# rtqichen/torchdiffeq

Measured on NVIDIA B200. Metric: trajectories/sec (dopri5, batch=65536 dim=128), higher is better.
Workload: dtype f32

## Files before the change

### include/tdq.h

```cpp
#ifndef TDQ_H_
#define TDQ_H_

#include <stddef.h>
#include <stdint.h>

#ifdef __cplusplus
extern "C" {
#endif

#define TDQ_ABI_VERSION 2

#define TDQ_MAX_STAGES 16
#define TDQ_MAX_K      (TDQ_MAX_STAGES + 1)
#define TDQ_MAX_SEGS   64
#define TDQ_MAX_RANKS  16

typedef enum {
    TDQ_OK = 0,
    TDQ_ERR_INVALID = 1,
    TDQ_ERR_CUDA = 2,
    TDQ_ERR_UNSUPPORTED = 3
} tdq_status;

typedef enum { TDQ_F32 = 0, TDQ_F64 = 1 } tdq_dtype;

typedef enum {
    TDQ_RUN_OK = 0,
    TDQ_RUN_DT_UNDERFLOW = 1,
    TDQ_RUN_NONFINITE = 2,
    TDQ_RUN_MAX_STEPS = 3,
    TDQ_RUN_EXCHANGE_TIMEOUT = 4
} tdq_run_status;

typedef struct {
    int32_t n_stages;
    int32_t order;
    int32_t fsal;
    int32_t reserved;
    double alpha[TDQ_MAX_STAGES];
    double beta[TDQ_MAX_STAGES][TDQ_MAX_K];
    double c_sol[TDQ_MAX_K];
    double c_err[TDQ_MAX_K];
    double c_mid[TDQ_MAX_K];
} tdq_tableau;

typedef struct {
    int32_t dtype;
    int32_t ratio_f64;
    double rtol, atol;
    double min_step, max_step;
    double safety, ifactor, dfactor;
    double t_sign;
    int64_t max_num_steps;
    int64_t n_global;
    void *ybuf[2];
    void *kbuf[2];
    int32_t always_fit;
    int32_t reserved;
    uint64_t loop_handle;
} tdq_options;

typedef struct {
    volatile uint64_t seq;
    volatile int32_t status;
    volatile int32_t accept;
    volatile int32_t done;
    volatile int32_t out_cursor;
    volatile int64_t n_accept, n_reject;
    volatile double t0, t1, dt;
    volatile double ratio;
    volatile double att_t0, att_dt;
    volatile double next_t0, next_dt;
    volatile int32_t on_jump_t;
    volatile int32_t par;
} tdq_mailbox;

int tdq_abi_version(void);
size_t tdq_sizeof(int32_t which);
const char *tdq_last_error(void);
int tdq_device_sm_count(int *out);

int tdq_tableau_get(const char *name, tdq_tableau *out);

int tdq_mailbox_create(tdq_mailbox **host_ptr, void **dev_ptr);
int tdq_mailbox_destroy(tdq_mailbox *host_ptr);

size_t tdq_ctrl_size(void);
size_t tdq_ctrl_tstage_offset(void);
size_t tdq_ctrl_taux_offset(void);

int tdq_ctrl_init(void *ctrl_dev, const tdq_tableau *tab, const tdq_options *opt, const double *t_out_dev,
                  double t_start, int32_t n_out, void *mailbox_dev, void *stream);

int tdq_ctrl_set_step_t(void *ctrl_dev, const double *step_t_dev, int32_t n, void *stream);
int tdq_ctrl_set_jump_t(void *ctrl_dev, const double *jump_t_dev, int32_t n, void *stream);

int64_t tdq_norm_table_fill(const int64_t *seg_offsets, const int64_t *seg_lens, int32_t n_seg, int64_t n,
                            int32_t dtype, int64_t *table_host, int64_t capacity_words);
size_t tdq_norm_partials_len(size_t n, int64_t n_chunks);

int tdq_scaled_sumsq(void *ctrl_dev, int32_t dtype, const void *x, const void *x2, const void *y0,
                     const double *rtol_vec, const double *atol_vec, const int64_t *table_dev, int64_t n_chunks,
                     int32_t table_aligned, int32_t n_seg, size_t n, double *partials, double *out, void *stream);
int tdq_initial_step_h0(void *ctrl_dev, int32_t dtype, const double *d0_sumsq, const double *d1_sumsq,
                        const int64_t *seg_counts_dev, int32_t n_seg, void *stream);
int tdq_initial_step_probe(void *ctrl_dev, int32_t dtype, void *y_probe, const void *y0, const void *f0,
                           size_t n, void *stream);
int tdq_initial_step_finish(void *ctrl_dev, int32_t dtype, const double *d2_sumsq,
                            const int64_t *seg_counts_dev, int32_t n_seg, void *stream);
int tdq_set_first_step(void *ctrl_dev, double first_step, void *stream);

int tdq_prepare_attempt(void *ctrl_dev, int32_t dtype, const double *y0_nonfinite_count_dev, void *stream);

int tdq_stage_combine(void *ctrl_dev, const tdq_tableau *tab, int32_t dtype, int32_t row, void *y_out,
                      const void *y0, const void *const *k, size_t n, void *stream);

int tdq_stage_combine_final(void *ctrl_dev, const tdq_tableau *tab, int32_t dtype, void *y1_out, void *err_out,
                            const void *y0, const void *const *k, size_t n, void *stream);

int tdq_error_norm_commit(void *ctrl_dev, int32_t dtype, const void *err_pre, const void *k_last, const void *y0,
                          const void *y1, const double *rtol_vec, const double *atol_vec, const int64_t *table_dev,
                          int64_t n_chunks, int32_t table_aligned, int32_t n_seg, size_t n, double *partials,
                          double *out, void *err_over_tol_out, void *stream);
int tdq_commit_candidates(void *ctrl_dev, int32_t dtype, const void *y1, const void *k_last, size_t n, void *stream);

int tdq_controller(void *ctrl_dev, int32_t dtype, const double *norm_in, const int64_t *seg_counts_dev,
                   int32_t n_seg, const void *ratio_dev, void *stream);

int tdq_interp_fit_eval(void *ctrl_dev, const tdq_tableau *tab, int32_t dtype, const void *y1, const void *const *k,
                        void *const *coeff, void *solution, size_t n, void *stream);
int tdq_interp_eval_at(void *ctrl_dev, int32_t dtype, const void *const *coeff, const double *t_dev, void *out,
                       size_t n, void *stream);
int tdq_poly_eval(int32_t dtype, const void *const *coeff, double x, void *out, size_t n, void *stream);
int tdq_ctrl_reset_interval(void *ctrl_dev, void *stream);

int tdq_loop_create(void *body_graph, void **loop_out, uint64_t *handle_out);
int tdq_loop_launch(void *loop, void *stream);
int tdq_loop_destroy(void *loop);
int tdq_ctrl_set_loop(void *ctrl_dev, uint64_t loop_handle, void *stream);

int tdq_rk4_stage(int32_t dtype, int32_t which, void *y_out, const void *y0, const void *k1,
                  const void *k2, const void *k3, const void *k4, const void *dt_dev,
                  const int64_t *step_dev, size_t n, void *stream);
int tdq_fixed_emit(int32_t dtype, void *y0, const void *y1, void *solution,
                   const int32_t *rec_begin_dev, const int32_t *out_idx_dev, const int32_t *mode_dev,
                   const void *slope_dev, int64_t *step_dev, const void *tstage_all_dev,
                   void *tstage_cur_dev, int64_t n_steps, size_t n, void *stream);

int tdq_fixed_final_emit(int32_t dtype, int32_t which, void *y0, const void *k1, const void *k2, const void *k3,
                         const void *k4, const void *dt_dev, void *solution, const int32_t *rec_begin_dev,
                         const int32_t *out_idx_dev, const int32_t *mode_dev, const void *slope_dev, int64_t *step_dev,
                         const void *tstage_all_dev, void *tstage_cur_dev, int64_t n_steps, size_t n, void *stream);

int tdq_lincomb(int32_t dtype, void *out, const void *base, const void *const *x, const double *coefs, int32_t n_terms,
                size_t n, void *stream);

int tdq_linear_supported(int32_t dtype, int32_t width);
size_t tdq_linear_weights_bytes(int32_t width);
int tdq_linear_prepare(int32_t dtype, const void *weight, int32_t width, void *planes, void *stream);
int tdq_linear_apply(int32_t dtype, const void *y, const void *planes, int32_t width, size_t n_rows, void *k_out,
                     void *stream);
int tdq_linear_stage(void *ctrl_dev, const tdq_tableau *tab, int32_t dtype, int32_t row, void *k_out, void *y1_out,
                     void *err_out, const void *y0, const void *const *k, const void *planes, int32_t width, size_t n,
                     void *stream);

int tdq_linear_attempt_supported(const tdq_tableau *tab, int32_t dtype, int32_t width);
int tdq_linear_attempt(void *ctrl_dev, const tdq_tableau *tab, int32_t dtype, void *const *k_out, void *y1_out, void *err_out,
                       const void *y0, const void *k0, const void *planes, int32_t width, size_t n, double *partials,
                       double *norm_out, const int64_t *seg_counts_dev, int32_t store_always, void *stream);

int tdq_fixed_emit_cubic(int32_t dtype, const void *y0, const void *y1, const void *f0, const void *f1, void *solution,
                         const int32_t *out_idx_dev, const void *coef_dev, int32_t rec_lo, int32_t rec_hi, size_t n,
                         void *stream);

typedef struct { unsigned char bytes[64]; } tdq_ipc_handle;
int tdq_xchg_create(void **dev_ptr, tdq_ipc_handle *handle_out);
int tdq_xchg_open(const tdq_ipc_handle *handle, void **peer_ptr);
int tdq_xchg_close(void *peer_ptr);
int tdq_xchg_destroy(void *dev_ptr);
int tdq_ctrl_set_exchange(void *ctrl_dev, const void *const *peer_ptrs, int32_t rank, int32_t world,
                          uint64_t epoch, void *stream);

int tdq_pack_segments(int32_t dtype, void *dst, const void *const *src, const int64_t *offsets,
                      const int64_t *lens, const double *scales, int32_t n_src, void *stream);

#ifdef __cplusplus
}
#endif
#endif
```

### torchdiffeq_b200/_engine.py

```python
import ctypes as C
import time

import torch

from . import _lib

_DTYPES = {torch.float32: _lib.TDQ_F32, torch.float64: _lib.TDQ_F64}


def _stream():
    return torch.cuda.current_stream().cuda_stream


_SOLVER_STREAMS = {}


def solver_stream(device):
    idx = device.index if device.index is not None else torch.cuda.current_device()
    st = _SOLVER_STREAMS.get(idx)
    if st is None:
        st = _SOLVER_STREAMS[idx] = torch.cuda.Stream(device=idx)
    return st


class on_solver_stream:

    def __init__(self, device):
        self.device = device

    def __enter__(self):
        self.cur = torch.cuda.current_stream(self.device)
        self.s = solver_stream(self.device)
        if self.cur == self.s:
            self.ctx = None
            return self
        self.s.wait_stream(self.cur)
        self.ctx = torch.cuda.stream(self.s)
        self.ctx.__enter__()
        return self

    def __exit__(self, *exc):
        if self.ctx is not None:
            self.ctx.__exit__(*exc)
            self.cur.wait_stream(self.s)
        return False

    def publish(self, *tensors):
        if self.ctx is not None:
            for t in tensors:
                if isinstance(t, torch.Tensor) and t.is_cuda:
                    t.record_stream(self.cur)


class _RetryWithCopies(Exception):
    """func handed back a buffer it had already returned for an earlier stage of the same attempt."""


class SolverFailure(AssertionError):
    """Raised for the reference's in-loop assertions (rk_common.py:247, :286, :287)."""


class Layout:

    def __init__(self, shapes, dtype):
        self.shapes = [torch.Size(s) for s in shapes]
        self.dtype = dtype
        vec = 16 // torch.empty((), dtype=dtype).element_size()
        self.offsets, self.lens = [], []
        off = 0
        for s in self.shapes:
            n = s.numel()
            self.offsets.append(off)
            self.lens.append(n)
            off += (n + vec - 1) // vec * vec
        self.n = off
        self.n_real = sum(self.lens)

    def flatten(self, tensors, out=None):
        flat = out if out is not None else torch.zeros(self.n, dtype=self.dtype, device=tensors[0].device)
        for t, o, l in zip(tensors, self.offsets, self.lens):
            flat[o:o + l].copy_(t.reshape(-1))
        return flat

    def views(self, flat, lead=()):
        return tuple(flat[..., o:o + l].view((*lead, *s)) for o, l, s in zip(self.offsets, self.lens, self.shapes))


def pack_pieces(lib, dt_code, dtype, buf, f, pieces):
    offs, lens, scales = pieces
    srcs, keep = [], []
    for p_, l in zip(f, lens):
        if p_ is None:
            srcs.append(None)
            continue
        if p_.dtype != dtype:
            p_ = p_.to(dtype)
        p_ = p_.reshape(-1)
        if not p_.is_contiguous():
            p_ = p_.contiguous()
        if p_.numel() != l:
            raise ValueError("func returned a piece of %d elements, expected %d" % (p_.numel(), l))
        keep.append(p_)
        srcs.append(p_.data_ptr())
    n_launch = 0
    for lo in range(0, len(srcs), _lib.TDQ_MAX_SEGS):
        hi = min(lo + _lib.TDQ_MAX_SEGS, len(srcs))
        _lib.check(lib.tdq_pack_segments(
            dt_code, buf.data_ptr(), _lib.ptr_array(srcs[lo:hi]), _lib.i64_array(offs[lo:hi]),
            _lib.i64_array(lens[lo:hi]), _lib.dbl_array(scales[lo:hi]), hi - lo, _stream()))
        n_launch += 1
    return n_launch


class AdaptiveEngine:

    def __init__(self, fn, n, dtype, device, method, *, rtol, atol, segs=None, t_sign=1.0,
                 pieces=None, min_step=0.0, max_step=float("inf"), first_step=None, step_t=None, jump_t=None,
                 safety=0.9, ifactor=10.0, dfactor=0.2, max_num_steps=2 ** 31 - 1,
                 rtol_vec=None, atol_vec=None, norm_fn=None, q_view=None,
                 graph="auto", run_ahead=2, reduce_fn=None, n_global=None, seg_counts_global=None,
                 agree_fn=None, exchange=None, callbacks=None, keep_interp=False, device_loop="auto", post_fn=None):
        if device.type != "cuda":
            raise _lib.TdqError("torchdiffeq_b200 runs on CUDA devices only (got %s); there is no CPU path" % device)
        if dtype not in _DTYPES:
            raise _lib.TdqError("unsupported state dtype %s (float32 and float64 are implemented)" % dtype)
        self.lib = _lib.load()
        self.fn = fn
        self.n = int(n)
        self.dtype = dtype
        self.device = device
        self.dt_code = _DTYPES[dtype]
        self.tab = _lib.tableau(method)
        self.S = self.tab.n_stages
        self.fsal = bool(self.tab.fsal)
        self.pieces = pieces
        self.first_step = first_step
        self.norm_fn = norm_fn
        self.q_view = q_view
        self.reduce_fn = reduce_fn
        self.agree_fn = agree_fn
        self.exchange = exchange
        self.post_fn = post_fn
        if exchange is not None and post_fn is None:
            self.agree_fn = None
        self.callbacks = callbacks or {}
        self.graph_opt = graph
        self.run_ahead = int(run_ahead)
        self.device_loop = device_loop
        self.keep_interp = bool(keep_interp)
        self.jump_t = jump_t
        if self.callbacks or (jump_t is not None and jump_t.numel() > 0):
            self.graph_opt = False
            self.run_ahead = 0

        segs = segs if segs is not None else [(0, self.n)]
        self.n_seg = len(segs)
        n_real = sum(int(l) for _, l in segs)
        counts = seg_counts_global if seg_counts_global is not None else [int(l) for _, l in segs]
        self.seg_counts = torch.tensor(counts, dtype=torch.int64, device=device)
        if len(segs) == 1 and int(segs[0][0]) == 0 and int(segs[0][1]) == self.n:
            self.norm_table, self.n_chunks, self.table_aligned = None, 0, 0
        else:
            words = _lib.norm_table(segs, self.n, _DTYPES[dtype])
            self.norm_table = torch.tensor(words, dtype=torch.int64, device=device)
            self.n_chunks, self.table_aligned = int(words[1]), int(words[3])

        self.rtol_vec = rtol_vec
        self.atol_vec = atol_vec
        vtol = rtol_vec is not None
        self.ratio_f64 = vtol or dtype == torch.float64
        self.opt = _lib.Options(
            dtype=self.dt_code, ratio_f64=1 if vtol else 0,
            rtol=float(rtol) if not vtol else 0.0, atol=float(atol) if not vtol else 0.0,
            min_step=float(min_step), max_step=float(max_step), safety=float(safety),
            ifactor=float(ifactor), dfactor=float(dfactor), t_sign=float(t_sign),
            max_num_steps=int(max_num_steps), n_global=int(n_global if n_global is not None else n_real))
        self.step_t = step_t

        kw = dict(dtype=dtype, device=device)
        self.ctrl = torch.zeros(self.lib.tdq_ctrl_size(), dtype=torch.uint8, device=device)
        o = self.lib.tdq_ctrl_tstage_offset()
        self.tstage = self.ctrl[o:o + 8 * _lib.TDQ_MAX_K].view(dtype)
        o = self.lib.tdq_ctrl_taux_offset()
        self.taux = self.ctrl[o:o + 32].view(dtype)
        self.ybuf = [torch.zeros(self.n, **kw) for _ in range(2)]
        self.kbuf = [torch.zeros(self.n, **kw) for _ in range(2)]
        self.opt.ybuf[0], self.opt.ybuf[1] = self.ybuf[0].data_ptr(), self.ybuf[1].data_ptr()
        self.opt.kbuf[0], self.opt.kbuf[1] = self.kbuf[0].data_ptr(), self.kbuf[1].data_ptr()
        self.opt.always_fit = 1 if self.keep_interp else 0
        self.ytmp = torch.zeros(self.n, **kw)
        self.y1 = torch.zeros(self.n, **kw)
        self.errp = torch.zeros(self.n, **kw)
        if self.keep_interp:
            self.coeff = [torch.zeros(self.n, **kw) for _ in range(5)]
            self.coeff_ptrs = _lib.ptr_array([c.data_ptr() for c in self.coeff])
        else:
            self.coeff, self.coeff_ptrs = [], None
        self.partials = torch.zeros(self.lib.tdq_norm_partials_len(self.n, self.n_chunks), dtype=torch.float64,
                                    device=device)
        self.norm_out = torch.zeros(self.n_seg + 1, dtype=torch.float64, device=device)
        self.dsum = [torch.zeros(self.n_seg + 1, dtype=torch.float64, device=device) for _ in range(3)]
        self.kslots = {}
        self.qbuf = None
        self.ratio_buf = None
        if norm_fn is not None:
            self.qbuf = torch.zeros(self.n, dtype=torch.float64 if vtol else dtype, device=device)
            self.ratio_buf = torch.zeros((), dtype=torch.float64 if self.ratio_f64 else dtype, device=device)
        self._own_ptrs = None
        self.mbox_host = C.POINTER(_lib.Mailbox)()
        mdev = C.c_void_p()
        _lib.check(self.lib.tdq_mailbox_create(C.byref(self.mbox_host), C.byref(mdev)))
        self.mbox_dev = mdev.value
        self.solution = None
        self._graph = None
        self._graph_failed = False
        self._graph_keep = None
        self._loop = None
        self._loop_handle = 0
        self._loop_failed = False
        self._always_copy = False
        self.linear = None
        self.capture_in_solve = True
        self.n_attempts = 0
        self.nfe = 0
        self.nfe_total = 0
        self.launches = 0
        self._graph_launches = 0

    def __del__(self):
        try:
            if self.mbox_host:
                torch.cuda.synchronize(self.device)
                self._drop_graph()
                self.lib.tdq_mailbox_destroy(self.mbox_host)
                self.mbox_host = None
        except Exception:
            pass

    def _call_fn(self, t, y, slot, taken=(), dst=None):
        self.nfe += 1
        f = self.fn(t, y)
        if isinstance(f, torch.Tensor):
            if f.dtype != self.dtype:
                f = f.to(self.dtype)
            f = f.reshape(-1)
            if f.numel() != self.n:
                raise ValueError("func returned %d elements for a state of %d" % (f.numel(), self.n))
            if f.data_ptr() in taken and not self._always_copy:
                self._always_copy = True
                raise _RetryWithCopies()
            if (self._always_copy or not f.is_contiguous() or (f.data_ptr() % 16) != 0 or self._aliases(f)
                    or f.data_ptr() in taken):
                buf = self._slot(slot)
                buf.copy_(f)
                f = buf
            return f
        buf = dst if dst is not None else self._slot(slot)
        self.launches += pack_pieces(self.lib, self.dt_code, self.dtype, buf, f, self.pieces)
        if self.post_fn is not None:
            self.post_fn(buf)
        return buf

    def set_linear(self, weight, whole_attempt=True, fused_controller=True):
        width, S = int(weight.shape[0]), self.S
        if self.pieces is not None or self.post_fn is not None or self.n % width:
            return False
        beta, c_err = self.tab.beta, self.tab.c_err
        for i in range(S):
            used = {j for j in range(i + 1) if beta[i][j] != 0.0}
            if self.fsal and i == S - 1:
                used |= {j for j in range(S) if c_err[j] != 0.0}
            if not 1 <= len(used) <= 8:
                return False
        planes = torch.empty(int(self.lib.tdq_linear_weights_bytes(width)), dtype=torch.uint8, device=self.device)
        whole = bool(whole_attempt) and bool(self.lib.tdq_linear_attempt_supported(C.byref(self.tab), self.dt_code, width))
        fold = (whole and self.norm_table is None and self.n_seg == 1 and self.rtol_vec is None and self.norm_fn is None)
        self.linear = dict(weight=weight, width=width, planes=planes, whole=whole, fold=fold, ctrl=bool(fused_controller),
                           k=[torch.zeros(self.n, dtype=self.dtype, device=self.device) for _ in range(S)])
        self._drop_graph()
        return True

    def _eval(self, t, y, slot, dst=None):
        if self.linear is None:
            return self._call_fn(t, y, slot, dst=dst)
        self.nfe += 1
        out = dst if dst is not None else self._slot(slot)
        L = self.linear
        self._launch(self.lib.tdq_linear_apply(self.dt_code, y.data_ptr(), L["planes"].data_ptr(), L["width"],
                                               self.n // L["width"], out.data_ptr(), _stream()))
        return out

    @property
    def y0w(self):
        return self.ybuf[self.mbox_host.contents.par & 1]

    @property
    def k0(self):
        return self.kbuf[self.mbox_host.contents.par & 1]

    def _drop_graph(self):
        if self._loop is not None:
            try:
                self.lib.tdq_loop_destroy(self._loop)
            except Exception:
                pass
        self._loop, self._loop_handle = None, 0
        self._graph, self._graph_keep = None, None

    def _launch(self, rc):
        _lib.check(rc)
        self.launches += 1

    def _slot(self, i):
        if i not in self.kslots:
            self.kslots[i] = torch.zeros(self.n, dtype=self.dtype, device=self.device)
        return self.kslots[i]

    def _aliases(self, f):
        if self._own_ptrs is None:
            own = self.ybuf + self.kbuf + [self.ytmp, self.y1, self.errp, self.solution] + self.coeff
            self._own_ptrs = {t.untyped_storage().data_ptr() for t in own}
        return f.untyped_storage().data_ptr() in self._own_ptrs

    def _reduce(self, buf):
        if self.reduce_fn is not None:
            self.reduce_fn(buf)

    def _sumsq(self, x, x2, out):
        self._launch(self.lib.tdq_scaled_sumsq(
            self.ctrl.data_ptr(), self.dt_code, x.data_ptr(), x2.data_ptr() if x2 is not None else None,
            None,
            self.rtol_vec.data_ptr() if self.rtol_vec is not None else None,
            self.atol_vec.data_ptr() if self.atol_vec is not None else None,
            self.norm_table.data_ptr() if self.norm_table is not None else None, self.n_chunks, self.table_aligned,
            self.n_seg, self.n, self.partials.data_ptr(), out.data_ptr(), _stream()))
        self._reduce(out)

    def _attempt_front(self):
        try:
            return self._attempt_front_once()
        except _RetryWithCopies:
            return self._attempt_front_once()

    def _attempt_front_once(self):
        lib, ctrl, tab, dc, st = self.lib, self.ctrl.data_ptr(), C.byref(self.tab), self.dt_code, _stream()
        S = self.S
        k = [None] * (S + 1)
        keep = []
        folded = False
        if self.linear is not None and self.linear["whole"]:
            L = self.linear
            for i in range(S):
                k[i + 1] = L["k"][i].data_ptr()
            folded = L["fold"]
            with_ctrl = folded and L["ctrl"] and (self.reduce_fn is None or self.exchange is not None)
            self._launch(lib.tdq_linear_attempt(ctrl, tab, dc, _lib.ptr_array(k), self.y1.data_ptr(), self.errp.data_ptr(),
                                                None, None, L["planes"].data_ptr(), L["width"], self.n,
                                                self.partials.data_ptr() if folded else None,
                                                self.norm_out.data_ptr() if folded else None,
                                                self.seg_counts.data_ptr() if with_ctrl else None,
                                                0 if folded else 1, st))
            self.nfe += S
            if with_ctrl:
                return k, _lib.ptr_array(k), keep
        elif self.linear is not None:
            L = self.linear
            for i in range(S):
                last = i == S - 1 and self.fsal
                out = L["k"][i]
                self._launch(lib.tdq_linear_stage(ctrl, tab, dc, i, out.data_ptr(),
                                                  self.y1.data_ptr() if last else None,
                                                  self.errp.data_ptr() if last else None, None, _lib.ptr_array(k),
                                                  L["planes"].data_ptr(), L["width"], self.n, st))
                self.nfe += 1
                k[i + 1] = out.data_ptr()
        for i in range(S if self.linear is None else 0):
            if i == S - 1 and self.fsal:
                out = self.y1
                self._launch(lib.tdq_stage_combine_final(ctrl, tab, dc, out.data_ptr(), self.errp.data_ptr(), None,
                                                         _lib.ptr_array(k), self.n, st))
            else:
                out = self.ytmp
                self._launch(lib.tdq_stage_combine(ctrl, tab, dc, i, out.data_ptr(), None, _lib.ptr_array(k), self.n,
                                                   st))
            f = self._call_fn(self.tstage[i], out, i + 1, taken=k)
            keep.append(f)
            k[i + 1] = f.data_ptr()
        if not self.fsal:
            self._launch(lib.tdq_stage_combine_final(ctrl, tab, dc, self.y1.data_ptr(), self.errp.data_ptr(), None,
                                                     _lib.ptr_array(k), self.n, st))
        kp = _lib.ptr_array(k)
        if not folded:
            self._launch(lib.tdq_error_norm_commit(
                ctrl, dc, self.errp.data_ptr(), k[S], None, self.y1.data_ptr(),
                self.rtol_vec.data_ptr() if self.rtol_vec is not None else None,
                self.atol_vec.data_ptr() if self.atol_vec is not None else None,
                self.norm_table.data_ptr() if self.norm_table is not None else None, self.n_chunks, self.table_aligned,
                self.n_seg, self.n, self.partials.data_ptr(), self.norm_out.data_ptr(),
                self.qbuf.data_ptr() if self.qbuf is not None else None, st))
        ratio_ptr = None
        if self.norm_fn is not None:
            r = self.norm_fn(self.q_view(self.qbuf))
            r = torch.as_tensor(r, device=self.device)
            self.ratio_buf.copy_(r.to(self.ratio_buf.dtype).reshape(()))
            ratio_ptr = self.ratio_buf.data_ptr()
        elif self.exchange is None:
            self._reduce(self.norm_out)
        self._launch(lib.tdq_controller(ctrl, dc, self.norm_out.data_ptr(), self.seg_counts.data_ptr(), self.n_seg,
                                      ratio_ptr, st))
        return k, kp, keep

    def _attempt_back(self, kp):
        self._launch(self.lib.tdq_interp_fit_eval(self.ctrl.data_ptr(), C.byref(self.tab), self.dt_code,
                                                  self.y1.data_ptr(), kp, self.coeff_ptrs, self.solution.data_ptr(),
                                                  self.n, _stream()))

    def _attempt(self):
        k, kp, keep = self._attempt_front()
        self._attempt_back(kp)
        return keep

    def _wait_seq(self, target):
        mb = self.mbox_host.contents
        spins = 0
        while mb.seq < target:
            spins += 1
            if spins > 2000:
                time.sleep(0)
                if spins % 20000 == 0 and torch.cuda.current_stream().query() and mb.seq < target:
                    raise _lib.TdqError("the device finished the queued attempts without reporting attempt %d (mailbox at %d)"
                                        % (target, mb.seq))
        return mb

    def _raise_if_failed(self, mb):
        s = mb.status
        if s == _lib.RUN_OK:
            return
        torch.cuda.current_stream().synchronize()
        if s == _lib.RUN_DT_UNDERFLOW:
            raise SolverFailure("underflow in dt {}".format(mb.next_dt))
        if s == _lib.RUN_NONFINITE:
            raise SolverFailure("non-finite values in state `y`: {}".format(self.y0w))
        if s == _lib.RUN_EXCHANGE_TIMEOUT:
            raise _lib.TdqError("a peer rank did not deliver its norm partials within 10 s (sharded solve)")
        if s == _lib.RUN_MAX_STEPS:
            raise SolverFailure("max_num_steps exceeded ({}>={})".format(self.opt.max_num_steps, self.opt.max_num_steps))
        raise SolverFailure("solver failed with status %d" % s)

    def _lockstep_mode(self):
        return bool(self.callbacks) or self.run_ahead == 0

    def _use_loop(self):
        return (self._loop is not None and not self._lockstep_mode() and self.agree_fn is None
                and self.norm_fn is None)

    def solve(self, y0_flat, t64, t_start=None):
        try:
            n_out = self._begin(y0_flat, t64, t_start, loop=self._use_loop())
            if n_out > 1:
                if self._lockstep_mode():
                    self._loop_lockstep()
                else:
                    self._loop_run_ahead()
        except BaseException:
            self.poisoned = True
            try:
                torch.cuda.current_stream().synchronize()
            except Exception:
                pass
            raise
        mb = self.mbox_host.contents
        self.n_accept, self.n_reject = int(mb.n_accept), int(mb.n_reject)
        self.n_attempts = self.n_accept + self.n_reject
        return self.solution

    def prime(self, y0_flat, t64, t_start=None):
        if self.graph_opt not in (True, "auto") or self._lockstep_mode():
            return False
        n_out = self._begin(y0_flat, t64, t_start)
        if n_out <= 1:
            return False
        self._warm_attempt()
        self._capture()
        torch.cuda.current_stream().synchronize()
        return self._graph is not None

    def _begin(self, y0_flat, t64, t_start=None, loop=False):
        lib = self.lib
        self.nfe_total += self.nfe
        self.nfe, self.launches = 0, 0
        n_out = int(t64.numel())
        self.t_out = t64.contiguous()
        if getattr(self, "solution", None) is None or self.solution.shape[0] != n_out:
            self.solution = torch.empty(n_out, self.n, dtype=self.dtype, device=self.device)
            self._drop_graph()
            self._own_ptrs = None
            loop = False
        self.solution[0].copy_(y0_flat)
        self.ybuf[0].copy_(y0_flat)
        st = _stream()
        mb = self.mbox_host.contents
        mb.seq, mb.status, mb.done, mb.par, mb.accept = 0, 0, 0, 0, 0
        mb.n_accept, mb.n_reject = 0, 0
        if t_start is None:
            t_start = float(t64[0])
        self.opt.loop_handle = self._loop_handle if loop else 0
        _lib.check(lib.tdq_ctrl_init(self.ctrl.data_ptr(), C.byref(self.tab), C.byref(self.opt),
                                     self.t_out.data_ptr(), float(t_start), n_out, self.mbox_dev, st))
        if self.exchange is not None:
            self.exchange.arm(self.ctrl.data_ptr(), st)
        if self.jump_t is not None and self.jump_t.numel() > 0:
            self._launch(lib.tdq_ctrl_set_jump_t(self.ctrl.data_ptr(), self.jump_t.data_ptr(),
                                                 int(self.jump_t.numel()), st))
        if self.step_t is not None and self.step_t.numel() > 0:
            self._launch(lib.tdq_ctrl_set_step_t(self.ctrl.data_ptr(), self.step_t.data_ptr(),
                                               int(self.step_t.numel()), st))
        dc, ctrl = self.dt_code, self.ctrl.data_ptr()
        if self.linear is not None:
            L = self.linear
            self._launch(lib.tdq_linear_prepare(dc, L["weight"].data_ptr(), L["width"], L["planes"].data_ptr(), st))

        f0 = self._eval(self.taux[0], self.ybuf[0], 0, dst=self.kbuf[0])
        if f0.data_ptr() != self.kbuf[0].data_ptr():
            self.kbuf[0].copy_(f0)
        del f0
        self._sumsq(self.ybuf[0], None, self.dsum[0])
        if self.first_step is None:
            if self.norm_fn is not None:
                self._initial_step_custom_norm()
            else:
                self._sumsq(self.kbuf[0], None, self.dsum[1])
                self._launch(lib.tdq_initial_step_h0(ctrl, dc, self.dsum[0].data_ptr(), self.dsum[1].data_ptr(),
                                                   self.seg_counts.data_ptr(), self.n_seg, st))
                self._launch(lib.tdq_initial_step_probe(ctrl, dc, self.ytmp.data_ptr(), None, None, self.n, st))
                f1 = self._eval(self.taux[1], self.ytmp, 1)
                self._sumsq(f1, self.kbuf[0], self.dsum[2])
                del f1
                self._launch(lib.tdq_initial_step_finish(ctrl, dc, self.dsum[2].data_ptr(),
                                                       self.seg_counts.data_ptr(), self.n_seg, st))
        else:
            self._launch(lib.tdq_set_first_step(ctrl, float(self.first_step), st))
        bad_ptr = self.dsum[0].data_ptr() + 8 * self.n_seg if n_out > 1 else None
        self._launch(lib.tdq_prepare_attempt(ctrl, dc, bad_ptr, st))
        return n_out

    def _lockstep_attempt(self, issued, mb):
        cb = self.callbacks
        if cb.get("callback_step") is not None:
            cb["callback_step"](*self._with_y(mb.next_t0, mb.next_dt))
        k, kp, keep = self._attempt_front()
        issued += 1
        mb = self._wait_seq(issued)
        self._raise_if_failed(mb)
        if cb:
            name = "callback_accept_step" if mb.accept else "callback_reject_step"
            if cb.get(name) is not None:
                cb[name](*self._with_y(mb.att_t0, mb.att_dt))
        jumped = bool(mb.accept) and bool(mb.on_jump_t)
        self._attempt_back(kp)
        del k, kp, keep
        if jumped:
            k0 = self.k0
            f = self._call_fn(self.taux[2], self.y0w, 0, dst=k0)
            if f.data_ptr() != k0.data_ptr():
                k0.copy_(f)
            del f
        return issued, mb

    def _loop_lockstep(self):
        issued = 0
        torch.cuda.current_stream().synchronize()
        mb = self.mbox_host.contents
        self._raise_if_failed(mb)
        while True:
            issued, mb = self._lockstep_attempt(issued, mb)
            if mb.done:
                break
        torch.cuda.current_stream().synchronize()

    def solve_dense(self, y0_flat, t64):
        n_out = self._begin(y0_flat, t64)
        torch.cuda.current_stream().synchronize()
        mb = self.mbox_host.contents
        self._raise_if_failed(mb)
        times, coeffs, issued = [float(t64[0])], [], 0
        while n_out > 1:
            issued, mb = self._lockstep_attempt(issued, mb)
            if mb.accept:
                times.append(float(mb.t1))
                coeffs.append([c.clone() for c in self.coeff])
            if mb.done:
                break
        torch.cuda.current_stream().synchronize()
        return self.solution, times, coeffs

    def solve_taped(self, y0_flat, t64, t_start=None):
        n_out = self._begin(y0_flat, t64, t_start)
        torch.cuda.current_stream().synchronize()
        mb = self.mbox_host.contents
        self._raise_if_failed(mb)
        tape, issued, cursor, first, jumped = [], 0, 1, True, None
        while n_out > 1:
            issued, mb = self._lockstep_attempt(issued, mb)
            if mb.accept:
                prev = (mb.par ^ 1) & 1
                k0 = self.kbuf[prev]
                tape.append(dict(t0=float(mb.att_t0), dt=float(mb.att_dt), y0=self.ybuf[prev].clone(), k0=k0.clone(),
                                 out_lo=cursor, out_hi=int(mb.out_cursor), first=first, jumped_into=jumped))
                cursor, first = int(mb.out_cursor), False
                jumped = True if mb.on_jump_t else None
            if mb.done:
                break
        torch.cuda.current_stream().synchronize()
        self.n_accept, self.n_reject = int(mb.n_accept), int(mb.n_reject)
        self.n_attempts = self.n_accept + self.n_reject
        return self.solution, tape

    def solve_until_event(self, y0_flat, t0, event_fn, tol):
        t64 = torch.tensor([float(t0), float("inf")], dtype=torch.float64, device=self.device)
        self._begin(y0_flat, t64, float(t0))
        torch.cuda.current_stream().synchronize()
        mb = self.mbox_host.contents
        self._raise_if_failed(mb)
        tt = lambda v: torch.tensor(v, dtype=torch.float64, device=self.device)
        t_cur = float(t0)
        if bool(event_fn(tt(t_cur), self.y0w) == 0):
            return t_cur, self.y0w.clone()
        sign0 = torch.sign(event_fn(tt(t_cur), self.y0w))
        issued = 0
        while bool(sign0 == torch.sign(event_fn(tt(t_cur), self.y0w))):
            issued, mb = self._lockstep_attempt(issued, mb)
            t_cur = mb.t1
        torch.cuda.current_stream().synchronize()
        self.n_accept, self.n_reject = int(mb.n_accept), int(mb.n_reject)
        self.n_attempts = self.n_accept + self.n_reject
        lo, hi = float(mb.t0), float(mb.t1)
        import math
        nitrs = int(math.ceil(math.log((hi - lo) / float(tol)) / math.log(2.0)))
        y_mid = torch.empty(self.n, dtype=self.dtype, device=self.device)

        def interp(t_eval):
            self._launch(self.lib.tdq_interp_eval_at(self.ctrl.data_ptr(), self.dt_code, self.coeff_ptrs,
                                                     tt(t_eval).data_ptr(), y_mid.data_ptr(), self.n, _stream()))
            return y_mid
        for _ in range(max(nitrs, 0)):
            t_mid = (hi + lo) / 2.0
            same = bool(sign0 == torch.sign(event_fn(tt(t_mid), interp(t_mid))))
            if same:
                lo = t_mid
            else:
                hi = t_mid
        event_t = (lo + hi) / 2.0
        return event_t, interp(event_t).clone()

    def _with_y(self, t0, dt):
        t0, dt = self._scalars(t0, dt)
        return t0, self.y0w, dt

    def _scalars(self, t0, dt):
        kw = dict(dtype=torch.float64, device=self.device)
        return torch.tensor(t0, **kw), torch.tensor(dt, **kw)

    def _loop_run_ahead(self):
        D = max(1, self.run_ahead)
        mb = self.mbox_host.contents
        issued = 0
        use_graph = self.graph_opt in (True, "auto") and not self._graph_failed and self.capture_in_solve
        if self._use_loop() and self.opt.loop_handle != 0:
            self._launch_loop()
            return
        if self._graph is None:
            if use_graph:
                self._warm_attempt()
                self._capture()
            else:
                self._attempt()
            issued += 1
            if self._use_loop():
                _lib.check(self.lib.tdq_ctrl_set_loop(self.ctrl.data_ptr(), self._loop_handle, _stream()))
                self._launch_loop(first=1)
                return
        while True:
            seen = mb.seq
            if mb.status != _lib.RUN_OK or mb.done:
                break
            if issued - seen > D:
                time.sleep(0)
                continue
            if self._graph is not None:
                self._graph.replay()
                self.nfe += self.S
                self.launches += self._graph_launches
            else:
                self._attempt()
            issued += 1
        if self.agree_fn is not None:
            target = self.agree_fn(issued)
            while issued < target:
                if self._graph is not None:
                    self._graph.replay()
                    self.nfe += self.S
                    self.launches += self._graph_launches
                else:
                    self._attempt()
                issued += 1
        mb = self._wait_seq(issued)
        self._raise_if_failed(mb)
        torch.cuda.current_stream().synchronize()

    def _launch_loop(self, first=0):
        _lib.check(self.lib.tdq_loop_launch(self._loop, _stream()))
        torch.cuda.current_stream().synchronize()
        mb = self.mbox_host.contents
        ran = int(mb.seq) - first
        self.nfe += self.S * ran
        self.launches += self._graph_launches * ran
        self._raise_if_failed(mb)

    def _warm_attempt(self):
        self._attempt()

    def _capture(self):
        last = None
        for _try in range(2):
            try:
                want_loop = (self.device_loop in (True, "auto") and not self._loop_failed and self.agree_fn is None
                             and self.norm_fn is None)
                g = torch.cuda.CUDAGraph(keep_graph=True) if want_loop else torch.cuda.CUDAGraph()
                nfe, launches = self.nfe, self.launches
                try:
                    with torch.cuda.graph(g, stream=solver_stream(self.device)):
                        keep = self._attempt()
                finally:
                    self._graph_launches = self.launches - launches
                    self.nfe, self.launches = nfe, launches
                self._graph, self._graph_keep = g, keep
                if want_loop:
                    self._make_loop(g)
                return
            except Exception as e:
                last = e
                self._graph = None
                torch.cuda.synchronize(self.device)
        self._graph_failed = True
        if self.graph_opt is True:
            raise last
        import warnings
        warnings.warn("torchdiffeq_b200: CUDA graph capture of the step body failed (%s: %s); "
                      "continuing with eager launches" % (type(last).__name__, last))

    def _make_loop(self, g):
        loop, handle = C.c_void_p(), C.c_uint64()
        try:
            _lib.check(self.lib.tdq_loop_create(C.c_void_p(g.raw_cuda_graph()), C.byref(loop), C.byref(handle)))
            self._loop, self._loop_handle = loop.value, int(handle.value)
        except Exception as e:
            self._loop, self._loop_handle, self._loop_failed = None, 0, True
            if self.device_loop is True:
                raise
            import warnings
            warnings.warn("torchdiffeq_b200: the captured step could not be wrapped into a device-side loop "
                          "(%s: %s); the host replays it instead" % (type(e).__name__, e))

    def _initial_step_custom_norm(self):
        T = self.dtype
        y0, f0 = self.ybuf[0], self.kbuf[0] * self.opt.t_sign
        if self.rtol_vec is not None:
            scale = self.atol_vec + torch.abs(y0) * self.rtol_vec
        else:
            scale = float(self.opt.atol) + torch.abs(y0) * float(self.opt.rtol)
        nf = lambda v: torch.as_tensor(self.norm_fn(self.q_view(v)), device=self.device).abs()
        d0, d1 = nf(y0 / scale), nf(f0 / scale)
        if d0 < 1e-5 or d1 < 1e-5:
            h0 = torch.tensor(1e-6, dtype=T, device=self.device)
        else:
            h0 = 0.01 * d0 / d1
        h0 = h0.abs()
        self.ytmp.copy_(y0 + h0 * f0)
        t0 = float(self.t_out[0])
        self.taux[1] = (torch.tensor(t0, dtype=torch.float64, device=self.device) + h0.double()).to(T) * self.opt.t_sign
        f1 = self._call_fn(self.taux[1], self.ytmp, 1) * self.opt.t_sign
        d2 = torch.abs(nf((f1 - f0) / scale) / h0)
        order = self.tab.order - 1
        if d1 <= 1e-15 and d2 <= 1e-15:
            h1 = torch.max(torch.tensor(1e-6, dtype=T, device=self.device), h0 * 1e-3)
        else:
            h1 = (0.01 / max(d1, d2)) ** (1. / float(order + 1))
        h1 = h1.abs()
        dt = float(torch.min(100 * h0, h1).to(torch.float64))
        self._launch(self.lib.tdq_set_first_step(self.ctrl.data_ptr(), dt, _stream()))
```

### torchdiffeq_b200/_lib.py

```python
import ctypes as C
import os

_HERE = os.path.dirname(os.path.abspath(__file__))
LIB_PATH = os.path.join(_HERE, "csrc", "libtdq.so")

TDQ_MAX_STAGES = 16
TDQ_MAX_K = TDQ_MAX_STAGES + 1
TDQ_MAX_SEGS = 64
TDQ_F32, TDQ_F64 = 0, 1
RUN_OK, RUN_DT_UNDERFLOW, RUN_NONFINITE, RUN_MAX_STEPS, RUN_EXCHANGE_TIMEOUT = 0, 1, 2, 3, 4
TDQ_MAX_RANKS = 16
ABI_VERSION = 2


class IpcHandle(C.Structure):
    _fields_ = [("bytes", C.c_ubyte * 64)]


class Tableau(C.Structure):
    _fields_ = [
        ("n_stages", C.c_int32), ("order", C.c_int32), ("fsal", C.c_int32), ("reserved", C.c_int32),
        ("alpha", C.c_double * TDQ_MAX_STAGES),
        ("beta", (C.c_double * TDQ_MAX_K) * TDQ_MAX_STAGES),
        ("c_sol", C.c_double * TDQ_MAX_K),
        ("c_err", C.c_double * TDQ_MAX_K),
        ("c_mid", C.c_double * TDQ_MAX_K),
    ]


class Options(C.Structure):
    _fields_ = [
        ("dtype", C.c_int32), ("ratio_f64", C.c_int32),
        ("rtol", C.c_double), ("atol", C.c_double),
        ("min_step", C.c_double), ("max_step", C.c_double),
        ("safety", C.c_double), ("ifactor", C.c_double), ("dfactor", C.c_double),
        ("t_sign", C.c_double),
        ("max_num_steps", C.c_int64), ("n_global", C.c_int64),
        ("ybuf", C.c_void_p * 2), ("kbuf", C.c_void_p * 2),
        ("always_fit", C.c_int32), ("reserved", C.c_int32),
        ("loop_handle", C.c_uint64),
    ]


class Mailbox(C.Structure):
    _fields_ = [
        ("seq", C.c_uint64),
        ("status", C.c_int32), ("accept", C.c_int32), ("done", C.c_int32), ("out_cursor", C.c_int32),
        ("n_accept", C.c_int64), ("n_reject", C.c_int64),
        ("t0", C.c_double), ("t1", C.c_double), ("dt", C.c_double),
        ("ratio", C.c_double), ("att_t0", C.c_double), ("att_dt", C.c_double),
        ("next_t0", C.c_double), ("next_dt", C.c_double),
        ("on_jump_t", C.c_int32), ("par", C.c_int32),
    ]


class TdqError(RuntimeError):
    pass


_vp, _i32, _i64, _sz, _dbl = C.c_void_p, C.c_int32, C.c_int64, C.c_size_t, C.c_double
_pp = C.POINTER(C.c_void_p)
_pi64 = C.POINTER(C.c_int64)
_pdbl = C.POINTER(C.c_double)
_ptab = C.POINTER(Tableau)

_SIGNATURES = {
    "tdq_abi_version": (C.c_int, []),
    "tdq_sizeof": (_sz, [_i32]),
    "tdq_last_error": (C.c_char_p, []),
    "tdq_device_sm_count": (C.c_int, [C.POINTER(C.c_int)]),
    "tdq_tableau_get": (C.c_int, [C.c_char_p, _ptab]),
    "tdq_mailbox_create": (C.c_int, [C.POINTER(C.POINTER(Mailbox)), _pp]),
    "tdq_mailbox_destroy": (C.c_int, [C.POINTER(Mailbox)]),
    "tdq_ctrl_size": (_sz, []),
    "tdq_ctrl_tstage_offset": (_sz, []),
    "tdq_ctrl_taux_offset": (_sz, []),
    "tdq_ctrl_init": (C.c_int, [_vp, _ptab, C.POINTER(Options), _vp, _dbl, _i32, _vp, _vp]),
    "tdq_ctrl_set_step_t": (C.c_int, [_vp, _vp, _i32, _vp]),
    "tdq_ctrl_set_jump_t": (C.c_int, [_vp, _vp, _i32, _vp]),
    "tdq_norm_table_fill": (_i64, [_pi64, _pi64, _i32, _i64, _i32, _pi64, _i64]),
    "tdq_norm_partials_len": (_sz, [_sz, _i64]),
    "tdq_scaled_sumsq": (C.c_int, [_vp, _i32, _vp, _vp, _vp, _vp, _vp, _vp, _i64, _i32, _i32, _sz, _vp, _vp, _vp]),
    "tdq_initial_step_h0": (C.c_int, [_vp, _i32, _vp, _vp, _vp, _i32, _vp]),
    "tdq_initial_step_probe": (C.c_int, [_vp, _i32, _vp, _vp, _vp, _sz, _vp]),
    "tdq_initial_step_finish": (C.c_int, [_vp, _i32, _vp, _vp, _i32, _vp]),
    "tdq_set_first_step": (C.c_int, [_vp, _dbl, _vp]),
    "tdq_prepare_attempt": (C.c_int, [_vp, _i32, _vp, _vp]),
    "tdq_stage_combine": (C.c_int, [_vp, _ptab, _i32, _i32, _vp, _vp, _pp, _sz, _vp]),
    "tdq_stage_combine_final": (C.c_int, [_vp, _ptab, _i32, _vp, _vp, _vp, _pp, _sz, _vp]),
    "tdq_error_norm_commit": (C.c_int, [_vp, _i32, _vp, _vp, _vp, _vp, _vp, _vp, _vp, _i64, _i32, _i32, _sz, _vp, _vp,
                                        _vp, _vp]),
    "tdq_commit_candidates": (C.c_int, [_vp, _i32, _vp, _vp, _sz, _vp]),
    "tdq_controller": (C.c_int, [_vp, _i32, _vp, _vp, _i32, _vp, _vp]),
    "tdq_interp_fit_eval": (C.c_int, [_vp, _ptab, _i32, _vp, _pp, _pp, _vp, _sz, _vp]),
    "tdq_interp_eval_at": (C.c_int, [_vp, _i32, _pp, _vp, _vp, _sz, _vp]),
    "tdq_poly_eval": (C.c_int, [_i32, _pp, _dbl, _vp, _sz, _vp]),
    "tdq_ctrl_reset_interval": (C.c_int, [_vp, _vp]),
    "tdq_loop_create": (C.c_int, [_vp, _pp, C.POINTER(C.c_uint64)]),
    "tdq_loop_launch": (C.c_int, [_vp, _vp]),
    "tdq_loop_destroy": (C.c_int, [_vp]),
    "tdq_ctrl_set_loop": (C.c_int, [_vp, C.c_uint64, _vp]),
    "tdq_rk4_stage": (C.c_int, [_i32, _i32, _vp, _vp, _vp, _vp, _vp, _vp, _vp, _vp, _sz, _vp]),
    "tdq_fixed_emit": (C.c_int, [_i32, _vp, _vp, _vp, _vp, _vp, _vp, _vp, _vp, _vp, _vp, _i64, _sz, _vp]),
    "tdq_fixed_final_emit": (C.c_int, [_i32, _i32, _vp, _vp, _vp, _vp, _vp, _vp, _vp, _vp, _vp, _vp, _vp, _vp, _vp, _vp,
                                       _i64, _sz, _vp]),
    "tdq_lincomb": (C.c_int, [_i32, _vp, _vp, _pp, _pdbl, _i32, _sz, _vp]),
    "tdq_linear_supported": (C.c_int, [_i32, _i32]),
    "tdq_linear_weights_bytes": (_sz, [_i32]),
    "tdq_linear_prepare": (C.c_int, [_i32, _vp, _i32, _vp, _vp]),
    "tdq_linear_apply": (C.c_int, [_i32, _vp, _vp, _i32, _sz, _vp, _vp]),
    "tdq_linear_stage": (C.c_int, [_vp, _ptab, _i32, _i32, _vp, _vp, _vp, _vp, _pp, _vp, _i32, _sz, _vp]),
    "tdq_linear_attempt_supported": (C.c_int, [_ptab, _i32, _i32]),
    "tdq_linear_attempt": (C.c_int, [_vp, _ptab, _i32, _pp, _vp, _vp, _vp, _vp, _vp, _i32, _sz, _vp, _vp, _vp, _i32, _vp]),
    "tdq_fixed_emit_cubic": (C.c_int, [_i32, _vp, _vp, _vp, _vp, _vp, _vp, _vp, _i32, _i32, _sz, _vp]),
    "tdq_pack_segments": (C.c_int, [_i32, _vp, _pp, _pi64, _pi64, _pdbl, _i32, _vp]),
    "tdq_xchg_create": (C.c_int, [_pp, C.POINTER(IpcHandle)]),
    "tdq_xchg_open": (C.c_int, [C.POINTER(IpcHandle), _pp]),
    "tdq_xchg_close": (C.c_int, [_vp]),
    "tdq_xchg_destroy": (C.c_int, [_vp]),
    "tdq_ctrl_set_exchange": (C.c_int, [_vp, _pp, _i32, _i32, C.c_uint64, _vp]),
}

EXPORTED_SYMBOLS = tuple(_SIGNATURES)

_lib = None


def load():
    global _lib
    if _lib is not None:
        return _lib
    if not os.path.exists(LIB_PATH):
        raise TdqError(
            "libtdq.so is not built (%s). Run `python -m torchdiffeq_b200.csrc.build` "
            "(or __graft_entry__.build()); there is no fallback path." % LIB_PATH)
    lib = C.CDLL(LIB_PATH)
    for name, (res, args) in _SIGNATURES.items():
        try:
            fn = getattr(lib, name)
        except AttributeError as e:
            raise TdqError("libtdq.so does not export %s; rebuild it" % name) from e
        fn.restype = res
        fn.argtypes = args
    if lib.tdq_abi_version() != ABI_VERSION:
        raise TdqError("libtdq.so ABI version mismatch")
    for which, st in ((0, Tableau), (1, Options), (2, Mailbox)):
        if lib.tdq_sizeof(which) != C.sizeof(st):
            raise TdqError("libtdq.so struct layout mismatch for %s; rebuild it" % st.__name__)
    _lib = lib
    return lib


def check(rc):
    if rc != 0:
        msg = load().tdq_last_error()
        raise TdqError("libtdq call failed (%d): %s" % (rc, msg.decode() if msg else "?"))


def tableau(name):
    t = Tableau()
    check(load().tdq_tableau_get(name.encode(), C.byref(t)))
    return t


def tableau_as_dict(name):
    t = tableau(name)
    S = t.n_stages
    return {
        "n_stages": S, "order": t.order, "fsal": bool(t.fsal),
        "alpha": [t.alpha[i] for i in range(S)],
        "beta": [[t.beta[i][j] for j in range(i + 1)] for i in range(S)],
        "c_sol": [t.c_sol[j] for j in range(S + 1)],
        "c_err": [t.c_err[j] for j in range(S + 1)],
        "c_mid": [t.c_mid[j] for j in range(S + 1)],
    }


def norm_table(segs, n, dt_code):
    lib = load()
    offs = i64_array([int(o) for o, _ in segs])
    lens = i64_array([int(l) for _, l in segs])
    words = lib.tdq_norm_table_fill(offs, lens, len(segs), int(n), dt_code, None, 0)
    if words < 0:
        check(1)
    buf = (C.c_int64 * words)()
    if lib.tdq_norm_table_fill(offs, lens, len(segs), int(n), dt_code, buf, words) != words:
        check(1)
    return list(buf)


def ptr_array(ptrs):
    arr = (C.c_void_p * len(ptrs))()
    for i, p in enumerate(ptrs):
        arr[i] = p
    return arr


def i64_array(vals):
    return (C.c_int64 * len(vals))(*vals)


def dbl_array(vals):
    return (C.c_double * len(vals))(*vals)
```

### torchdiffeq_b200/csrc/tdq_attempt.cu

```cuda
#include "tdq_shape.cuh"
#include "tdq_tc.cuh"
#include "tdq_ctrl_dev.cuh"

#include <type_traits>

namespace {

using namespace tdq_tc;

constexpr int LD = 128;
constexpr int AT_ROWS = 16;
constexpr int AT_PLANE = AT_ROWS * LD * 2;
constexpr int AT_STAGE = 3 * AT_PLANE;
constexpr int AT_AUX = 2048;
constexpr int AT_Y0 = AT_ROWS * LD * 4;
constexpr int at_smem(int G) { return G * (AT_STAGE + AT_Y0) + AT_AUX + 1024; }
constexpr int AT_TMEM_COLS = 512;
constexpr int AT_COL_W = 256;
constexpr int AT_MAX_S = 7;
constexpr uint32_t IDESC16 = tc_idesc(AT_ROWS) | (1u << 16);

constexpr uint32_t AT_LBO = 128, AT_SBO = 2048;
__device__ __forceinline__ uint64_t make_desc_mn(uint32_t saddr) {
    return (uint64_t)((saddr & 0x3FFFFu) >> 4) | ((uint64_t)(AT_LBO >> 4) << 16) | ((uint64_t)(AT_SBO >> 4) << 32) | (1ull << 46);
}
__device__ __forceinline__ void sts_v4(uint32_t addr, uint32_t a, uint32_t b, uint32_t c, uint32_t d) {
    asm volatile("st.shared.v4.b32 [%0], {%1, %2, %3, %4};" :: "r"(addr), "r"(a), "r"(b), "r"(c), "r"(d) : "memory");
}

template <int N>
__device__ __forceinline__ uint32_t dep16(const float (&a)[N], uint32_t zero) {
    uint32_t x = 0;
#pragma unroll
    for (int r = 0; r < N; ++r) x ^= __float_as_uint(a[r]);
    return x & zero;
}
__device__ __forceinline__ void tmem_ld8(uint32_t taddr, uint32_t (&r)[8]) {
    asm volatile("tcgen05.ld.sync.aligned.32x32b.x8.b32 {%0,%1,%2,%3,%4,%5,%6,%7}, [%8];"
                 : "=r"(r[0]), "=r"(r[1]), "=r"(r[2]), "=r"(r[3]), "=r"(r[4]), "=r"(r[5]), "=r"(r[6]), "=r"(r[7])
                 : "r"(taddr) : "memory");
}
template <int N> __device__ __forceinline__ void tmem_ldn(uint32_t taddr, uint32_t (&r)[N]);
template <> __device__ __forceinline__ void tmem_ldn<16>(uint32_t taddr, uint32_t (&r)[16]) { tmem_ld16(taddr, r); }
template <> __device__ __forceinline__ void tmem_ldn<8>(uint32_t taddr, uint32_t (&r)[8]) { tmem_ld8(taddr, r); }
__device__ __forceinline__ bool elect_one() {
    uint32_t pred = 0;
    asm volatile("{\n\t.reg .pred p;\n\telect.sync _|p, 0xffffffff;\n\t@p mov.s32 %0, 1;\n\t}\n" : "+r"(pred));
    return pred != 0;
}
__device__ __forceinline__ void sts_f32(uint32_t addr, float v) { asm volatile("st.shared.f32 [%0], %1;" :: "r"(addr), "f"(v) : "memory"); }
__device__ __forceinline__ float lds_f32(uint32_t addr) {
    float v;
    asm volatile("ld.shared.f32 %0, [%1];" : "=f"(v) : "r"(addr) : "memory");
    return v;
}

struct AttOut {
    float *k[AT_MAX_S + 1];
    float *y1, *err;
};

__host__ __device__ constexpr int popc_below(unsigned mask, int j) {
    int n = 0;
    for (int b = 0; b < j; ++b) n += (mask >> b) & 1u;
    return n;
}

template <int S, unsigned long long RM, unsigned EM, int G, int RT, bool CTRL, int ACCS>
__global__ void __launch_bounds__(G * 128 * (16 / RT), 1)
k_linear_attempt(TdqCtrl *c, const float *y0, const float *k0, AttOut out, const uint32_t *__restrict__ wt,
                 double *partials, double *norm_out, const int64_t *seg_counts, int store_always, size_t n_rows_sz) {
    if (c->halt) {
        if (CTRL && blockIdx.x == 0) tdq_ctrl_dev::controller_block<float, G * 128 * (16 / RT)>(c, norm_out, seg_counts, 1, nullptr);
        return;
    }
    extern __shared__ uint8_t smem_raw[];
    uint8_t *smem = reinterpret_cast<uint8_t *>((reinterpret_cast<uintptr_t>(smem_raw) + 1023) & ~(uintptr_t)1023);
    constexpr int AT_GROUPS = G, HN = AT_ROWS / RT, WPG = 4 * HN, AT_THREADS = G * 128 * HN;
    uint8_t *aux = smem + G * (AT_STAGE + AT_Y0);
    uint64_t *bars = reinterpret_cast<uint64_t *>(aux);
    uint32_t *tmem_slot = reinterpret_cast<uint32_t *>(aux + 32);
    int *s_flag = reinterpret_cast<int *>(aux + 40);
    float *s_cr = reinterpret_cast<float *>(aux + 64);
    float *s_ce = s_cr + AT_MAX_S * 8;
    double *s_red = reinterpret_cast<double *>(aux + 512);
    const int tid = threadIdx.x, lane = tid & 31;
    const int warp = __shfl_sync(0xffffffffu, tid >> 5, 0);
    const int n_rows = (int)n_rows_sz;
    const uint32_t bar0 = smem_u32(bars);

    if (warp == 0) {
        asm volatile("tcgen05.alloc.cta_group::1.sync.aligned.shared::cta.b32 [%0], %1;" :: "r"(smem_u32(tmem_slot)), "n"(AT_TMEM_COLS) : "memory");
        asm volatile("tcgen05.relinquish_alloc_permit.cta_group::1.sync.aligned;" ::: "memory");
    }
    if (tid == 32) {
#pragma unroll
        for (int g = 0; g < AT_GROUPS; ++g) mbar_init(bar0 + 8 * g, 1);
        asm volatile("fence.mbarrier_init.release.cluster;" ::: "memory");
    }
    if (tid >= 64 && tid < 64 + AT_MAX_S * 8) {
        const int i = (tid - 64) >> 3, m = (tid - 64) & 7;
        s_cr[i * 8 + m] = (i < S) ? (float)c->coef[i][m] : 0.f;
        if (i == 0) s_ce[m] = (float)c->ecoef[m];
    }
    fence_before();
    __syncthreads();
    fence_after();
    const uint32_t tmem = __shfl_sync(0xffffffffu, *tmem_slot, 0);

    const int g = warp / WPG, wl = warp % WPG, e = wl & 3, h = wl >> 2, f = e * 32 + lane;
    const uint32_t lane_base = tmem + ((uint32_t)(e * 32) << 16);
    {
#pragma unroll 1
        for (int ch = warp >> 2; ch < 6; ch += AT_THREADS / 128) {
            const int pl = ch >> 1, c0 = (ch & 1) * 32;
            uint32_t r[32];
            const uint4 *src = reinterpret_cast<const uint4 *>(wt + ((size_t)pl * LD + f) * 64 + c0);
#pragma unroll
            for (int j = 0; j < 8; ++j) {
                const uint4 v = src[j];
                r[4 * j] = v.x; r[4 * j + 1] = v.y; r[4 * j + 2] = v.z; r[4 * j + 3] = v.w;
            }
            tmem_st32(lane_base + AT_COL_W + pl * 64 + c0, r);
        }
        asm volatile("tcgen05.wait::st.sync.aligned;" ::: "memory");
    }
    fence_before();
    __syncthreads();
    fence_after();

    if (y0 == nullptr) y0 = reinterpret_cast<const float *>(c->y0_cur);
    if (k0 == nullptr) k0 = reinterpret_cast<const float *>(c->k0_cur);
    y0 = tdq_detach(y0, n_rows_sz);
    k0 = tdq_detach(k0, n_rows_sz);
    const bool fold = partials != nullptr;
    float *ycand = nullptr, *kcand = nullptr;
    if (fold && c->ybuf[0] != nullptr) {
        ycand = tdq_detach(reinterpret_cast<float *>(c->ybuf[c->par ^ 1]), n_rows_sz);
        kcand = tdq_detach(reinterpret_cast<float *>(c->kbuf[c->par ^ 1]), n_rows_sz);
    }
    bool store = store_always != 0 || c->always_fit != 0;
    if (!store) {
        const int cur = c->out_cursor;
        store = cur < c->n_out && !(c->t_out[cur] > c->att_t1);
    }
    const float rtolT = (float)c->rtol, atolT = (float)c->atol;
    constexpr int EK = popc_below(EM, S);
    const float ecS = s_ce[EK];

    uint8_t *stage = smem + g * AT_STAGE;
    const uint32_t sy0 = smem_u32(smem + AT_GROUPS * AT_STAGE + g * AT_Y0) + (uint32_t)(h * RT * LD + f) * 4;
    const uint32_t stage_u32 = smem_u32(stage);
    const uint32_t bar = bar0 + 8 * g;
    constexpr int ACOLS = 32 * ACCS;
    const uint32_t acc0 = tmem + g * ACOLS;
    uint32_t phase = 0;
    const uint32_t st_f = stage_u32 + (uint32_t)f * 16 + (uint32_t)(h * (RT / 8)) * AT_SBO;

    const int tiles = (n_rows + AT_ROWS - 1) / AT_ROWS;
    const int workers = (int)gridDim.x * AT_GROUPS;
    double acc = 0.0;
    int nbad = 0;
    const uint32_t zero32 = (uint32_t)(n_rows_sz >> 63);

    constexpr int KEEP = S < 4 ? S : 4;
    constexpr int NACC = S - KEEP;
    auto row_mask = [](int i) -> unsigned { return (unsigned)((RM >> (8 * i)) & 0xffull); };
    auto do_tile = [&](auto full_tag, const int t) {
        constexpr bool FULL = decltype(full_tag)::value;
        const int row0 = t * AT_ROWS;
        const int rows_here = FULL ? RT : n_rows - row0 - h * RT;
        const size_t base = (size_t)(row0 + h * RT) * LD + f;
        float K[KEEP][RT];
        float A[NACC > 0 ? NACC : 1][RT];
        float AE[RT], PRE[RT], KN[RT], Y1[RT];
        {
            float Y0[RT];
#pragma unroll
            for (int r = 0; r < RT; ++r) {
                Y0[r] = 0.f;
                KN[r] = 0.f;
                if (FULL || r < rows_here) {
                    Y0[r] = __ldcs(y0 + base + (size_t)r * LD);
                    KN[r] = __ldcs(k0 + base + (size_t)r * LD);
                }
            }
#pragma unroll
            for (int r = 0; r < RT; ++r) sts_f32(sy0 + r * LD * 4, Y0[r]);
        }
#pragma unroll
        for (int i = 0; i < S; ++i) {
            const unsigned mask = row_mask(i);
            const bool last = i == S - 1;
            const bool has_prefix = (mask & ((1u << i) - 1u)) != 0u, has_new = ((mask >> i) & 1u) != 0u;
            const float c_new = has_new ? s_cr[i * 8 + popc_below(mask, i)] : 0.f;
            if (i < KEEP) {
#pragma unroll
                for (int r = 0; r < RT; ++r) K[i < KEEP ? i : 0][r] = KN[r];
            }
#pragma unroll
            for (int r8 = 0; r8 < RT; r8 += 8) {
                uint32_t H[4], M[4], L[4];
#pragma unroll
                for (int r = r8; r < r8 + 8; r += 2) {
                    float yv[2];
#pragma unroll
                    for (int q = 0; q < 2; ++q) {
                        const float pre = i < KEEP ? PRE[r + q] : A[i >= KEEP ? i - KEEP : 0][r + q];
                        float sum;
                        if (has_prefix && has_new) sum = pre + KN[r + q] * c_new;
                        else if (has_prefix) sum = pre;
                        else sum = KN[r + q] * c_new;
                        yv[q] = lds_f32(sy0 + (r + q) * LD * 4) + sum;
                        if (last) Y1[r + q] = yv[q];
                    }
                    split2(yv[0], yv[1], H[(r - r8) >> 1], M[(r - r8) >> 1], L[(r - r8) >> 1]);
                }
                sts_v4(st_f + (r8 >> 3) * AT_SBO, H[0], H[1], H[2], H[3]);
                sts_v4(st_f + AT_PLANE + (r8 >> 3) * AT_SBO, M[0], M[1], M[2], M[3]);
                sts_v4(st_f + 2 * AT_PLANE + (r8 >> 3) * AT_SBO, L[0], L[1], L[2], L[3]);
            }
            fence_async_smem();
            fence_before();
            asm volatile("bar.sync %0, %1;" :: "r"(g + 1), "n"(WPG * 32) : "memory");
            if (wl == g % 4 && elect_one()) {
                fence_after();
                constexpr int NPROD = 6;
                constexpr int PW[NPROD] = {1, 2, 0, 1, 0, 0}, PY[NPROD] = {1, 0, 2, 0, 1, 0};
#pragma unroll
                for (int p = 0; p < NPROD; ++p) {
#pragma unroll
                    for (int ks = 0; ks < 8; ++ks) {
                        const uint32_t dcol = acc0 + (ks % ACCS) * 32 + (p == NPROD - 1 ? 0 : 16);
                        mma_ts(dcol, tmem + AT_COL_W + PW[p] * 64 + ks * 8, make_desc_mn(stage_u32 + PY[p] * AT_PLANE + ks * 2 * AT_LBO), IDESC16,
                               (p == 0 || p == NPROD - 1) && ks < ACCS ? 0u : 1u);
                    }
                }
                mma_commit(bar);
            }
            __syncwarp();
            uint32_t dep = 0;
            if (i + 1 < KEEP && i + 1 < S) {
                const unsigned mn = row_mask(i + 1);
                bool first = true;
#pragma unroll
                for (int j = 0; j <= i; ++j) {
                    if ((mn >> j) & 1u) {
                        const float cj = s_cr[(i + 1) * 8 + popc_below(mn, j)];
#pragma unroll
                        for (int r = 0; r < RT; ++r) {
                            const float p = K[j < KEEP ? j : 0][r] * cj;
                            PRE[r] = first ? p : PRE[r] + p;
                        }
                        first = false;
                    }
                }
                if (!first) dep |= dep16(PRE, zero32);
            }
            if (i == KEEP - 1) {
#pragma unroll
                for (int r = 0; r < RT; ++r) {
#pragma unroll
                    for (int qrow = KEEP; qrow < S; ++qrow) {
                        const unsigned mq = row_mask(qrow);
                        float a_ = 0.f;
                        bool first = true;
#pragma unroll
                        for (int j = 0; j <= i; ++j) {
                            if ((mq >> j) & 1u) {
                                const float p = K[j < KEEP ? j : 0][r] * s_cr[qrow * 8 + popc_below(mq, j)];
                                a_ = first ? p : a_ + p;
                                first = false;
                            }
                        }
                        A[qrow - KEEP][r] = a_;
                    }
                    float e_ = 0.f;
                    bool first = true;
#pragma unroll
                    for (int j = 0; j <= i; ++j) {
                        if ((EM >> j) & 1u) {
                            const float p = K[j < KEEP ? j : 0][r] * s_ce[popc_below(EM, j)];
                            e_ = first ? p : e_ + p;
                            first = false;
                        }
                    }
                    AE[r] = e_;
                }
#pragma unroll
                for (int qrow = KEEP; qrow < S; ++qrow) dep |= dep16(A[qrow - KEEP], zero32);
                dep |= dep16(AE, zero32);
            }
            if (i >= KEEP) {
#pragma unroll
                for (int qrow = i + 1; qrow < S; ++qrow) {
                    const unsigned mq = row_mask(qrow);
                    if ((mq >> i) & 1u) {
                        const float cj = s_cr[qrow * 8 + popc_below(mq, i)];
                        const bool started = (mq & ((1u << i) - 1u)) != 0u;
#pragma unroll
                        for (int r = 0; r < RT; ++r) {
                            const float p = KN[r] * cj;
                            A[qrow - KEEP][r] = started ? A[qrow - KEEP][r] + p : p;
                        }
                    }
                }
                if ((EM >> i) & 1u) {
                    const float cj = s_ce[popc_below(EM, i)];
                    const bool started = (EM & ((1u << i) - 1u)) != 0u;
#pragma unroll
                    for (int r = 0; r < RT; ++r) {
                        const float p = KN[r] * cj;
                        AE[r] = started ? AE[r] + p : p;
                    }
                }
#pragma unroll
                for (int qrow = i + 1; qrow < S; ++qrow) dep |= dep16(A[qrow - KEEP], zero32);
                dep |= dep16(AE, zero32);
            }
            if (last) {
#pragma unroll
                for (int r = 0; r < RT; ++r) {
                    const float y1v = Y1[r];
                    if (FULL || r < rows_here) {
                        if (!isfinite(y1v)) nbad += 1;
                        const size_t o = base + (size_t)r * LD;
                        if (ycand) ycand[o] = y1v;
                        if (store) {
                            out.y1[o] = y1v;
                            out.err[o] = AE[r];
                        }
                    }
                    Y1[r] = Ar<float>::add(atolT, Ar<float>::mul(rtolT, Ar<float>::max_nan(fabsf(lds_f32(sy0 + r * LD * 4)), fabsf(y1v))));
                }
                dep |= dep16(Y1, zero32);
            }
            mbar_wait(bar + dep, phase);
            phase ^= 1u;
            fence_after();
            {
                uint32_t tq[RT];
#pragma unroll
                for (int a_ = 0; a_ < 2 * ACCS; ++a_) {
                    const int col = (a_ < ACCS ? a_ * 32 + 16 : (a_ - ACCS) * 32) + h * RT;
                    tmem_ldn<RT>(lane_base + (uint32_t)(g * ACOLS + col), tq);
                    asm volatile("tcgen05.wait::ld.sync.aligned;" ::: "memory");
#pragma unroll
                    for (int r = 0; r < RT; ++r) KN[r] = a_ == 0 ? __uint_as_float(tq[r]) : KN[r] + __uint_as_float(tq[r]);
                }
            }
            if (store) {
#pragma unroll
                for (int r = 0; r < RT; ++r)
                    if (FULL || r < rows_here) out.k[i + 1][base + (size_t)r * LD] = KN[r];
            }
            if (last) {
#pragma unroll
                for (int r = 0; r < RT; ++r) {
                    if (FULL || r < rows_here) {
                        if (kcand) kcand[base + (size_t)r * LD] = KN[r];
                        if (fold) {
                            const float num = Ar<float>::add(AE[r], Ar<float>::mul(KN[r], ecS));
                            const float q = Ar<float>::div(num, Y1[r]);
                            acc += (double)Ar<float>::mul(q, q);
                        }
                    }
                }
            }
        }
    };
#pragma unroll 1
    for (int t = g * (int)gridDim.x + (int)blockIdx.x; t < tiles; t += workers) {
        {
            const int tn = t + workers, pr = lane & 15;
            const long long prow = (long long)tn * AT_ROWS + h * RT + pr;
            if (tn < tiles && pr < RT && prow < (long long)n_rows) {
                const float *pp = (lane < 16 ? y0 : k0) + (size_t)prow * LD + e * 32;
                asm volatile("prefetch.global.L2 [%0];" :: "l"(pp));
            }
        }
        if (n_rows - t * AT_ROWS >= AT_ROWS) do_tile(std::true_type{}, t);
        else do_tile(std::false_type{}, t);
    }
    const double bad = (double)nbad;

    if (fold) {
        const double wa = warp_sum(acc), wb = warp_sum(bad);
        if (lane == 0) {
            s_red[warp] = wa;
            s_red[32 + warp] = wb;
        }
    }
    fence_before();
    __syncthreads();
    if (warp == 0) {
        fence_after();
        asm volatile("tcgen05.dealloc.cta_group::1.sync.aligned.b32 %0, %1;" :: "r"(tmem), "n"(AT_TMEM_COLS) : "memory");
    }
    if (!fold) return;
    const int P = (int)gridDim.x;
    double *p_sum = partials + 2, *p_bad = p_sum + P;
    unsigned int *ticket = reinterpret_cast<unsigned int *>(partials);
    if (tid == 0) {
        double a = 0.0, b = 0.0;
        for (int w = 0; w < AT_THREADS / 32; ++w) {
            a += s_red[w];
            b += s_red[32 + w];
        }
        p_sum[blockIdx.x] = a;
        p_bad[blockIdx.x] = b;
        __threadfence();
        const unsigned int tk = atomicAdd(ticket, 1u);
        *s_flag = (tk == gridDim.x - 1) ? 1 : 0;
    }
    __syncthreads();
    if (!*s_flag) return;
    __threadfence();
    if (warp == 0) {
        double a = 0.0, b = 0.0;
        for (int i = lane; i < P; i += 32) {
            a += __ldcg(&p_sum[i]);
            b += __ldcg(&p_bad[i]);
        }
        a = warp_sum(a);
        b = warp_sum(b);
        if (lane == 0) {
            norm_out[0] = a;
            norm_out[1] = b;
            *ticket = 0;
        }
    }
    if (CTRL) {
        __threadfence();
        __syncthreads();
        tdq_ctrl_dev::controller_block<float, AT_THREADS>(c, norm_out, seg_counts, 1, nullptr);
    }
}

constexpr unsigned long long RM_DOPRI5 = 0x01ull | (0x03ull << 8) | (0x07ull << 16) | (0x0full << 24) | (0x1full << 32) | (0x3dull << 40);
constexpr unsigned long long RM_BOSH3 = 0x01ull | (0x02ull << 8) | (0x07ull << 16);

template <int S, unsigned long long RM, unsigned EM, int G, int RT, bool CTRL, int ACCS>
int launch_attempt_g(TdqCtrl *c, const float *y0, const float *k0, const AttOut &out, const uint32_t *wt, double *partials,
                     double *norm_out, const int64_t *seg_counts, int store_always, size_t n_rows, cudaStream_t st) {
    auto kern = k_linear_attempt<S, RM, EM, G, RT, CTRL, ACCS>;
    constexpr int AT_SMEM = at_smem(G);
    if (cudaFuncSetAttribute(kern, cudaFuncAttributeMaxDynamicSharedMemorySize, AT_SMEM) != cudaSuccess) return -2;
    const size_t tiles = (n_rows + AT_ROWS - 1) / AT_ROWS;
    size_t grid = (tiles + G - 1) / G;
    const size_t cap = (size_t)tdq_sm_count();
    if (grid > cap) grid = cap;
    if (grid == 0) grid = 1;
    kern<<<(unsigned)grid, G * 128 * (AT_ROWS / RT), AT_SMEM, st>>>(c, y0, k0, out, wt, partials, norm_out, seg_counts, store_always, n_rows);
    return 0;
}

template <int S, unsigned long long RM, unsigned EM>
int launch_attempt(TdqCtrl *c, const float *y0, const float *k0, const AttOut &out, const uint32_t *wt, double *partials,
                   double *norm_out, const int64_t *seg_counts, int store_always, size_t n_rows, cudaStream_t st) {
#define TDQ_GO(G_, RT_, A_) (seg_counts ? launch_attempt_g<S, RM, EM, G_, RT_, true, A_>(c, y0, k0, out, wt, partials, norm_out, seg_counts, store_always, n_rows, st) \
                                        : launch_attempt_g<S, RM, EM, G_, RT_, false, A_>(c, y0, k0, out, wt, partials, norm_out, seg_counts, store_always, n_rows, st))
    return TDQ_GO(4, 16, 1);
#undef TDQ_GO
}

bool attempt_masks(const TdqHostShape &hs, unsigned long long *rm, unsigned *em) {
    const int S = hs.n_stages;
    if (!hs.fsal || S < 2 || S > AT_MAX_S) return false;
    *rm = 0;
    *em = 0;
    for (int i = 0; i < S; ++i) {
        unsigned m = 0;
        for (int q = 0; q < hs.row_nnz[i]; ++q) {
            if (hs.row_idx[i][q] > i) return false;
            m |= 1u << hs.row_idx[i][q];
        }
        if (m == 0) return false;
        *rm |= (unsigned long long)m << (8 * i);
    }
    bool has_S = false;
    for (int q = 0; q < hs.err_nnz; ++q) {
        if (hs.err_idx[q] == S) has_S = true;
        else *em |= 1u << hs.err_idx[q];
    }
    return has_S && hs.err_idx[hs.err_nnz - 1] == S;
}

}

extern "C" {

int tdq_linear_attempt_supported(const tdq_tableau *tab, int32_t dtype, int32_t width) {
    if (!tab || dtype != TDQ_F32 || width != LD) return 0;
    TdqHostShape hs;
    tdq_shape_from_tableau(tab, &hs);
    unsigned long long rm;
    unsigned em;
    if (!attempt_masks(hs, &rm, &em)) return 0;
    const int S = hs.n_stages;
    return ((S == 6 && rm == RM_DOPRI5 && em == 0x3du) || (S == 3 && rm == RM_BOSH3 && em == 0x07u)) ? 1 : 0;
}

int tdq_linear_attempt(void *ctrl_dev, const tdq_tableau *tab, int32_t dtype, void *const *k_out, void *y1_out, void *err_out,
                       const void *y0, const void *k0, const void *planes, int32_t width, size_t n, double *partials,
                       double *norm_out, const int64_t *seg_counts_dev, int32_t store_always, void *stream) {
    TDQ_REQUIRE(ctrl_dev && tab && k_out && y1_out && err_out && planes, "null argument");
    TDQ_REQUIRE(dtype == TDQ_F32 && width == LD, "the fused linear field is float32, width 128");
    TDQ_REQUIRE(n % (size_t)width == 0, "state size is not a multiple of the field width");
    TDQ_REQUIRE((partials == nullptr) == (norm_out == nullptr), "partials and norm_out go together");
    TDQ_REQUIRE(seg_counts_dev == nullptr || partials != nullptr, "the controller step needs the folded error norm");
    const size_t n_rows = n / (size_t)width;
    TDQ_REQUIRE(n_rows < ((size_t)1 << 31) - 64, "too many rows");
    TdqHostShape hs;
    tdq_shape_from_tableau(tab, &hs);
    unsigned long long rm = 0;
    unsigned em = 0;
    TDQ_REQUIRE(attempt_masks(hs, &rm, &em), "the whole-attempt kernel takes FSAL tableaus of at most 7 stages");
    const int S = hs.n_stages;
    AttOut out;
    memset(&out, 0, sizeof(out));
    for (int i = 1; i <= S; ++i) {
        TDQ_REQUIRE(k_out[i] != nullptr, "missing stage slot");
        out.k[i] = (float *)k_out[i];
    }
    out.y1 = (float *)y1_out;
    out.err = (float *)err_out;
    if (n_rows == 0) return TDQ_OK;
    TdqCtrl *c = (TdqCtrl *)ctrl_dev;
    const uint32_t *wt = (const uint32_t *)planes;
    cudaStream_t st = (cudaStream_t)stream;
    int rc = -1;
    if (S == 6 && rm == RM_DOPRI5 && em == 0x3du)
        rc = launch_attempt<6, RM_DOPRI5, 0x3du>(c, (const float *)y0, (const float *)k0, out, wt, partials, norm_out, seg_counts_dev, store_always, n_rows, st);
    else if (S == 3 && rm == RM_BOSH3 && em == 0x07u)
        rc = launch_attempt<3, RM_BOSH3, 0x07u>(c, (const float *)y0, (const float *)k0, out, wt, partials, norm_out, seg_counts_dev, store_always, n_rows, st);
    TDQ_REQUIRE(rc != -1, "no whole-attempt kernel for this tableau (tdq_linear_attempt_supported)");
    TDQ_REQUIRE(rc == 0, "launch configuration failed");
    TDQ_CHECK_CUDA(cudaGetLastError());
    return TDQ_OK;
}

}
```

### torchdiffeq_b200/csrc/tdq_common.cuh

```cuda
#pragma once

#include <cuda_runtime.h>
#include <math_constants.h>
#include <stdint.h>
#include <string.h>

#include "tdq.h"

#define TDQ_ROWS (TDQ_MAX_STAGES + 1)

struct TdqCtrl {
    int32_t dtype, n_stages, order, fsal;
    int32_t ratio_f64, n_out, n_step_t, next_step_index;
    int32_t row_nnz[TDQ_ROWS];
    int32_t row_idx[TDQ_ROWS][TDQ_MAX_K];
    int32_t err_nnz, mid_nnz;
    int32_t err_idx[TDQ_MAX_K], mid_idx[TDQ_MAX_K];
    double alpha[TDQ_MAX_STAGES];
    double beta[TDQ_ROWS][TDQ_MAX_K];
    double c_err[TDQ_MAX_K], c_mid[TDQ_MAX_K];
    double rtol, atol;
    double min_step, max_step, safety, ifactor, dfactor, t_sign;
    int64_t max_num_steps, n_global;
    const double *t_out;
    const double *step_t;
    const double *jump_t;
    int32_t n_jump_t, next_jump_index, on_jump_t, pad_jump;
    tdq_mailbox *mbox;
    void *xpeer[TDQ_MAX_RANKS];
    unsigned long long xepoch;
    int32_t xrank, xworld;
    double t0, t1, dt;
    double att_t0, att_dt, att_t1;
    double ratio, h0;
    int32_t on_step_t, accept, status, done;
    int32_t halt, out_cursor, emit_lo, emit_hi;
    int64_t n_accept, n_reject, n_steps_interval;
    uint64_t seq;
    void *ybuf[2], *kbuf[2];
    const void *y0_cur, *k0_cur;
    const void *y0_prev, *k0_prev;
    int32_t par, always_fit, fit_now, y0_bad;
    unsigned long long loop_handle;
    double coef[TDQ_ROWS][TDQ_MAX_K];
    double ecoef[TDQ_MAX_K];
    double fit_mcoef[TDQ_MAX_K];
    double fit_sdt;
    double att_dtT;
    alignas(16) unsigned char tstage[8 * TDQ_MAX_K];
    alignas(16) unsigned char taux[8 * 4];
};

struct TdqXBuf {
    double vals[4][TDQ_MAX_RANKS][TDQ_MAX_SEGS + 2];
    unsigned long long flags[4][TDQ_MAX_RANKS];
};

template <typename T> struct Ar;
template <> struct Ar<float> {
    static __device__ __forceinline__ float mul(float a, float b) { return __fmul_rn(a, b); }
    static __device__ __forceinline__ float add(float a, float b) { return __fadd_rn(a, b); }
    static __device__ __forceinline__ float sub(float a, float b) { return __fsub_rn(a, b); }
    static __device__ __forceinline__ float div(float a, float b) { return __fdiv_rn(a, b); }
    static __device__ __forceinline__ float abs(float a) { return fabsf(a); }
    static __device__ __forceinline__ float max_nan(float a, float b) {
        return (a != a || b != b) ? CUDART_NAN_F : fmaxf(a, b);
    }
    static __device__ __forceinline__ bool finite(float a) { return isfinite(a); }
};
template <> struct Ar<double> {
    static __device__ __forceinline__ double mul(double a, double b) { return __dmul_rn(a, b); }
    static __device__ __forceinline__ double add(double a, double b) { return __dadd_rn(a, b); }
    static __device__ __forceinline__ double sub(double a, double b) { return __dsub_rn(a, b); }
    static __device__ __forceinline__ double div(double a, double b) { return __ddiv_rn(a, b); }
    static __device__ __forceinline__ double abs(double a) { return fabs(a); }
    static __device__ __forceinline__ double max_nan(double a, double b) {
        return (a != a || b != b) ? CUDART_NAN : fmax(a, b);
    }
    static __device__ __forceinline__ bool finite(double a) { return isfinite(a); }
};

template <typename T> struct Vec;
template <> struct alignas(16) Vec<float> {
    static constexpr int N = 4;
    float v[4];
};
template <> struct alignas(16) Vec<double> {
    static constexpr int N = 2;
    double v[2];
};

template <typename T> __device__ __forceinline__ Vec<T> ld_stream(const T *p);
template <> __device__ __forceinline__ Vec<float> ld_stream<float>(const float *p) {
    Vec<float> r;
    asm volatile("ld.global.L1::no_allocate.v4.f32 {%0,%1,%2,%3}, [%4];"
                 : "=f"(r.v[0]), "=f"(r.v[1]), "=f"(r.v[2]), "=f"(r.v[3]) : "l"(p));
    return r;
}
template <> __device__ __forceinline__ Vec<double> ld_stream<double>(const double *p) {
    Vec<double> r;
    asm volatile("ld.global.L1::no_allocate.v2.f64 {%0,%1}, [%2];"
                 : "=d"(r.v[0]), "=d"(r.v[1]) : "l"(p));
    return r;
}
template <typename T> __device__ __forceinline__ void st_vec(T *p, const Vec<T> &x);
template <> __device__ __forceinline__ void st_vec<float>(float *p, const Vec<float> &x) {
    asm volatile("st.global.v4.f32 [%0], {%1,%2,%3,%4};"
                 :: "l"(p), "f"(x.v[0]), "f"(x.v[1]), "f"(x.v[2]), "f"(x.v[3]) : "memory");
}
template <> __device__ __forceinline__ void st_vec<double>(double *p, const Vec<double> &x) {
    asm volatile("st.global.v2.f64 [%0], {%1,%2};" :: "l"(p), "d"(x.v[0]), "d"(x.v[1]) : "memory");
}

template <typename P>
__device__ __forceinline__ P *tdq_detach(P *p, size_t n) {
    return reinterpret_cast<P *>(reinterpret_cast<uintptr_t>(p) + (n >> 63));
}

struct KPtrs {
    const void *p[TDQ_MAX_K];
};
struct KPtrsMut {
    void *p[TDQ_MAX_K];
};

__device__ __forceinline__ double warp_sum(double v) {
#pragma unroll
    for (int o = 16; o > 0; o >>= 1) v += __shfl_down_sync(0xffffffffu, v, o);
    return v;
}
template <int THREADS> __device__ __forceinline__ double block_sum(double v, double *smem ) {
    const int lane = threadIdx.x & 31, w = threadIdx.x >> 5;
    v = warp_sum(v);
    __syncthreads();
    if (lane == 0) smem[w] = v;
    __syncthreads();
    double r = 0.0;
    if (w == 0) {
        r = (lane < THREADS / 32) ? smem[lane] : 0.0;
        r = warp_sum(r);
    }
    return r;
}

void tdq_set_error(const char *fmt, ...);
#define TDQ_CHECK_CUDA(expr)                                                              \
    do {                                                                                  \
        cudaError_t _e = (expr);                                                          \
        if (_e != cudaSuccess) {                                                          \
            tdq_set_error("%s failed: %s (%s:%d)", #expr, cudaGetErrorString(_e), __FILE__, __LINE__); \
            return TDQ_ERR_CUDA;                                                          \
        }                                                                                 \
    } while (0)
#define TDQ_REQUIRE(cond, msg)                                                            \
    do {                                                                                  \
        if (!(cond)) {                                                                    \
            tdq_set_error("%s: %s", __func__, msg);                                       \
            return TDQ_ERR_INVALID;                                                       \
        }                                                                                 \
    } while (0)

static inline bool tdq_aligned16(const void *p) { return (reinterpret_cast<uintptr_t>(p) & 15u) == 0; }
```

### torchdiffeq_b200/csrc/tdq_ctrl_dev.cuh

```cuda
#pragma once

#include "tdq_common.cuh"

namespace tdq_ctrl_dev {

template <typename T> __device__ __forceinline__ T prev_repr(T t);
template <> __device__ __forceinline__ float prev_repr<float>(float t) { return nextafterf(t, __fsub_rn(t, 1.0f)); }
template <> __device__ __forceinline__ double prev_repr<double>(double t) { return nextafter(t, __dsub_rn(t, 1.0)); }

template <typename T> __device__ __forceinline__ T next_repr(T t);
template <> __device__ __forceinline__ float next_repr<float>(float t) { return nextafterf(t, __fadd_rn(t, 1.0f)); }
template <> __device__ __forceinline__ double next_repr<double>(double t) { return nextafter(t, __dadd_rn(t, 1.0)); }

template <typename T> __device__ __forceinline__ void store_T(unsigned char *raw, int i, T v) {
    reinterpret_cast<T *>(raw)[i] = v;
}

template <typename T> __device__ void prepare_scalar(TdqCtrl &c) {
    if (c.halt) return;
    if (c.n_steps_interval >= c.max_num_steps) {
        c.status = TDQ_RUN_MAX_STEPS;
        c.halt = 1;
        return;
    }
    double dt = c.dt;
    if (!isfinite(dt)) dt = c.min_step;
    dt = fmin(fmax(dt, c.min_step), c.max_step);
    const double t0 = c.t1;
    double t1 = t0 + dt;
    c.att_t0 = t0;
    c.att_dt = dt;
    if (!(t0 + dt > t0)) {
        c.status = TDQ_RUN_DT_UNDERFLOW;
        c.halt = 1;
        return;
    }
    if (c.y0_bad) {
        c.status = TDQ_RUN_NONFINITE;
        c.halt = 1;
        return;
    }
    c.on_step_t = 0;
    if (c.n_step_t > 0) {
        const double nxt = c.step_t[c.next_step_index];
        if (t0 < nxt && nxt < t0 + dt) {
            c.on_step_t = 1;
            t1 = nxt;
            dt = t1 - t0;
        }
    }
    c.on_jump_t = 0;
    if (c.n_jump_t > 0) {
        const double nxt = c.jump_t[c.next_jump_index];
        if (t0 < nxt && nxt < t0 + dt) {
            c.on_jump_t = 1;
            c.on_step_t = 0;
            t1 = nxt;
            dt = t1 - t0;
        }
    }
    c.att_dt = dt;
    c.att_t1 = t1;
    c.att_dtT = (double)(T)dt;
}

template <typename T> __device__ void prepare_tables(TdqCtrl &c, int tid, int nthreads) {
    if (c.halt) return;
    using A = Ar<T>;
    const T t0T = (T)c.att_t0, dtT = (T)c.att_dt, t1T = (T)c.att_t1;
    const T sgn = (T)c.t_sign;
    const int S = c.n_stages;
    for (int i = tid; i < S; i += nthreads) {
        const T a = (T)c.alpha[i];
        T ti;
        if (a == (T)1) ti = prev_repr<T>(t1T);
        else ti = A::add(t0T, A::mul(a, dtT));
        store_T<T>(c.tstage, i, A::mul(sgn, ti));
    }
    const int rows = c.fsal ? S : S + 1;
    for (int e = tid; e < rows * TDQ_MAX_K; e += nthreads) {
        const int r = e / TDQ_MAX_K, m = e % TDQ_MAX_K;
        if (m < c.row_nnz[r]) c.coef[r][m] = (double)A::mul(sgn, A::mul((T)c.beta[r][m], dtT));
    }
    for (int m = tid; m < c.err_nnz; m += nthreads)
        c.ecoef[m] = (double)A::mul(sgn, A::mul(dtT, (T)c.c_err[m]));
}

template <typename T> __device__ void prepare_attempt(TdqCtrl &c) {
    prepare_scalar<T>(c);
    prepare_tables<T>(c, 0, 1);
}

template <typename T, int THREADS>
__device__ double block_norm_from_sums(const TdqCtrl &c, const double *sums, const int64_t *counts, int n_seg,
                                       double *smem ) {
    double best = 0.0;
    int nan = 0;
    for (int s = threadIdx.x; s < n_seg; s += THREADS) {
        const double cnt = counts ? (double)counts[s] : (double)c.n_global;
        if (cnt <= 0.0) continue;
        double r = sqrt(sums[s] / cnt);
        if (!c.ratio_f64) r = (double)(T)r;
        if (r != r) nan = 1;
        if (r > best) best = r;
    }
#pragma unroll
    for (int o = 16; o > 0; o >>= 1) {
        const double ob = __shfl_down_sync(0xffffffffu, best, o);
        const int on = __shfl_down_sync(0xffffffffu, nan, o);
        if (ob > best) best = ob;
        nan |= on;
    }
    const int lane = threadIdx.x & 31, w = threadIdx.x >> 5;
    __syncthreads();
    if (lane == 0) smem[w] = nan ? CUDART_NAN : best;
    __syncthreads();
    if (threadIdx.x == 0) {
        double b = 0.0;
        bool bn = false;
        for (int i = 0; i < THREADS / 32; ++i) {
            const double v = smem[i];
            if (v != v) bn = true;
            else if (v > b) b = v;
        }
        smem[THREADS / 32] = bn ? CUDART_NAN : b;
    }
    __syncthreads();
    return smem[THREADS / 32];
}

static __device__ void write_mailbox(TdqCtrl &c, double fin_t0, double fin_dt, int jumped = 0) {
    c.seq += 1;
    tdq_mailbox *m = c.mbox;
    if (!m) return;
    if (c.loop_handle != 0ull && !c.halt) return;
    m->status = c.status;
    m->accept = c.accept;
    m->done = c.done;
    m->out_cursor = c.out_cursor;
    m->n_accept = c.n_accept;
    m->n_reject = c.n_reject;
    m->t0 = c.t0;
    m->t1 = c.t1;
    m->dt = c.dt;
    m->ratio = c.ratio;
    m->att_t0 = fin_t0;
    m->att_dt = fin_dt;
    m->next_t0 = c.att_t0;
    m->next_dt = c.att_dt;
    m->on_jump_t = jumped;
    m->par = c.par;
    __threadfence_system();
    m->seq = c.seq;
}

template <typename T>
__device__ void controller(TdqCtrl &c, const double *norm_in, int n_seg, const void *ratio_dev, double ratio_pre) {
    if (c.halt) {
        c.accept = 0;
        c.fit_now = 0;
        c.emit_lo = c.emit_hi;
        write_mailbox(c, c.att_t0, c.att_dt);
        return;
    }
    using A = Ar<T>;
    double ratio;
    if (ratio_dev) {
        ratio = c.ratio_f64 ? *reinterpret_cast<const double *>(ratio_dev)
                            : (double)*reinterpret_cast<const T *>(ratio_dev);
        ratio = fabs(ratio);
    } else {
        ratio = ratio_pre;
    }
    const bool y1_nonfinite = norm_in && norm_in[n_seg] > 0.0;
    if (y1_nonfinite && !ratio_dev) ratio = CUDART_NAN;
    c.ratio = ratio;

    const double dt = c.att_dt;
    bool accept = ratio <= 1.0;
    if (dt > c.max_step) accept = false;
    if (dt <= c.min_step) accept = true;
    c.accept = accept ? 1 : 0;

    if (accept) {
        c.t0 = c.att_t0;
        c.t1 = c.att_t1;
        c.n_accept += 1;
        c.y0_prev = c.y0_cur;
        c.k0_prev = c.k0_cur;
        c.par ^= 1;
        c.y0_cur = c.ybuf[c.par];
        c.k0_cur = c.kbuf[c.par];
        if (c.on_step_t && c.next_step_index != c.n_step_t - 1) c.next_step_index += 1;
        if (c.on_jump_t) {
            if (c.next_jump_index != c.n_jump_t - 1) c.next_jump_index += 1;
            store_T<T>(c.taux, 2, A::mul((T)c.t_sign, next_repr<T>((T)c.att_t1)));
        }
        const T dtT = (T)c.att_dtT, sgn = (T)c.t_sign;
        c.fit_sdt = (double)A::mul(sgn, dtT);
        for (int m = 0; m < c.mid_nnz; ++m)
            c.fit_mcoef[m] = (double)A::mul(sgn, A::mul(dtT, (T)c.c_mid[m]));
        if (y1_nonfinite) {
            c.status = TDQ_RUN_NONFINITE;
            c.halt = 1;
        }
    } else {
        c.t0 = c.att_t0;
        c.t1 = c.att_t0;
        c.n_reject += 1;
    }

    double dt_next;
    if (ratio == 0.0) {
        dt_next = dt * c.ifactor;
    } else {
        const double dfac = (ratio < 1.0) ? 1.0 : c.dfactor;
        const double expo = 1.0 / (double)c.order;
        const double cand = c.safety / pow(ratio, expo);
        double inner = (cand != cand || dfac != dfac) ? CUDART_NAN : fmax(cand, dfac);
        double factor = (inner != inner) ? CUDART_NAN : fmin(c.ifactor, inner);
        dt_next = dt * factor;
    }
    if (dt_next == dt_next) dt_next = fmin(fmax(dt_next, c.min_step), c.max_step);
    c.dt = dt_next;

    c.emit_lo = c.out_cursor;
    c.n_steps_interval += 1;
    if (accept) {
        int cur = c.out_cursor;
        while (cur < c.n_out && !(c.t_out[cur] > c.t1)) ++cur;
        if (cur != c.out_cursor) c.n_steps_interval = 0;
        c.out_cursor = cur;
    }
    c.emit_hi = c.out_cursor;
    c.fit_now = (accept && (c.always_fit || c.emit_hi > c.emit_lo)) ? 1 : 0;
    if (c.out_cursor >= c.n_out) {
        c.done = 1;
        c.halt = 1;
    }
    const double fin_t0 = c.att_t0, fin_dt = c.att_dt;
    const int jumped = (accept && c.on_jump_t) ? 1 : 0;
    prepare_scalar<T>(c);
    write_mailbox(c, fin_t0, fin_dt, jumped);
}

static_assert(sizeof(TdqCtrl) % 8 == 0, "control block must be a whole number of 8-byte words");
static_assert(sizeof(TdqCtrl) <= 40 * 1024, "control block must fit static shared memory");

template <typename T, int THREADS>
__device__ void controller_block(TdqCtrl *c, const double *norm_in, const int64_t *cnt, int n_seg, const void *ratio_dev) {
    __shared__ __align__(16) unsigned char raw[sizeof(TdqCtrl)];
    constexpr int kWords = (int)(sizeof(TdqCtrl) / 8);
    unsigned long long *sw = reinterpret_cast<unsigned long long *>(raw);
    const unsigned long long *gw = reinterpret_cast<const unsigned long long *>(c);
    for (int i = threadIdx.x; i < kWords; i += THREADS) sw[i] = gw[i];
    __syncthreads();
    TdqCtrl &sc = *reinterpret_cast<TdqCtrl *>(raw);
    __shared__ double xsum[TDQ_MAX_SEGS + 2];
    __shared__ int xfail;
    if (sc.xworld > 1 && !sc.halt && norm_in != nullptr && ratio_dev == nullptr && n_seg <= TDQ_MAX_SEGS) {
        const int R = sc.xworld, me = sc.xrank, nv = n_seg + 1;
        const int par = (int)(((sc.xepoch & 1ull) << 1) | (sc.seq & 1ull));
        const unsigned long long want = (sc.xepoch << 32) | (sc.seq + 1ull);
        if (threadIdx.x == 0) xfail = 0;
        __syncthreads();
        if ((int)threadIdx.x < R) {
            const int t = threadIdx.x;
            TdqXBuf *peer = reinterpret_cast<TdqXBuf *>(sc.xpeer[t]);
            for (int i = 0; i < nv; ++i) peer->vals[par][me][i] = norm_in[i];
            __threadfence_system();
            asm volatile("st.release.sys.global.u64 [%0], %1;" :: "l"(&peer->flags[par][me]), "l"(want) : "memory");
            TdqXBuf *mine = reinterpret_cast<TdqXBuf *>(sc.xpeer[me]);
            unsigned long long seen = 0, t0 = 0, now = 0;
            asm volatile("mov.u64 %0, %%globaltimer;" : "=l"(t0));
            do {
                asm volatile("ld.acquire.sys.global.u64 %0, [%1];" : "=l"(seen) : "l"(&mine->flags[par][t]) : "memory");
                if (seen == want) break;
                asm volatile("mov.u64 %0, %%globaltimer;" : "=l"(now));
            } while (now - t0 < 10000000000ull);
            if (seen != want) atomicExch(&xfail, 1);
        }
        __syncthreads();
        if (threadIdx.x == 0) {
            if (xfail) {
                sc.status = TDQ_RUN_EXCHANGE_TIMEOUT;
                sc.halt = 1;
            } else {
                const TdqXBuf *mine = reinterpret_cast<const TdqXBuf *>(sc.xpeer[me]);
                for (int i = 0; i < nv; ++i) {
                    double a = 0.0;
                    for (int r = 0; r < R; ++r) a += __ldcg(&mine->vals[par][r][i]);
                    xsum[i] = a;
                }
            }
        }
        __syncthreads();
        norm_in = xsum;
    }
    __shared__ double nsm[THREADS / 32 + 1];
    double ratio_pre = 0.0;
    if (!sc.halt && ratio_dev == nullptr)
        ratio_pre = block_norm_from_sums<T, THREADS>(sc, norm_in, cnt, n_seg, nsm);
    __shared__ int was_halted;
    if (threadIdx.x == 0) {
        was_halted = sc.halt;
        controller<T>(sc, norm_in, n_seg, ratio_dev, ratio_pre);
    }
    __syncthreads();
    if (!was_halted) prepare_tables<T>(sc, threadIdx.x, THREADS);
    __syncthreads();
    unsigned long long *go = reinterpret_cast<unsigned long long *>(c);
    for (int i = threadIdx.x; i < kWords; i += THREADS) go[i] = sw[i];
    if (threadIdx.x == 0 && sc.loop_handle != 0ull)
        cudaGraphSetConditional((cudaGraphConditionalHandle)sc.loop_handle, sc.halt ? 0u : 1u);
}

}
```

### torchdiffeq_b200/odeint.py

```python
import collections
import warnings

import torch

from . import _lib
from ._engine import AdaptiveEngine, Layout, on_solver_stream
from ._fixed import FixedGridEngine, grid_from_step_size

ADAPTIVE_METHODS = ("dopri5", "dopri8", "tsit5", "bosh3", "fehlberg2", "adaptive_heun")
FIXED_METHODS = ("euler", "midpoint", "heun2", "heun3", "rk4")
ADAMS_METHODS = {"explicit_adams": False, "implicit_adams": True, "fixed_adams": True}
REFERENCE_METHODS = (
    "dopri8", "dopri5", "tsit5", "bosh3", "fehlberg2", "adaptive_heun", "euler", "midpoint", "heun2", "heun3",
    "rk4", "explicit_adams", "implicit_adams", "implicit_euler", "implicit_midpoint", "trapezoid", "radauIIA3",
    "gl4", "radauIIA5", "gl6", "sdirk2", "trbdf2", "fixed_adams", "scipy_solver")

_CALLBACK_NAMES = ["callback_step", "callback_accept_step", "callback_reject_step"]
_ADJOINT_CALLBACK_NAMES = [name + "_adjoint" for name in _CALLBACK_NAMES]
_ADAPTIVE_OPTIONS = {"min_step", "max_step", "first_step", "step_t", "jump_t", "safety", "ifactor", "dfactor",
                     "max_num_steps", "dtype", "norm"}
_FIXED_OPTIONS = {"step_size", "grid_constructor", "interp", "perturb", "norm"}
_ADAMS_OPTIONS = _FIXED_OPTIONS | {"max_iters", "max_order"}
_OUR_OPTIONS = {"graph", "run_ahead", "process_group", "cache", "exchange", "device_loop", "fused_linear", "fused_attempt", "fused_controller"}


def _rms_norm(tensor):
    return tensor.abs().pow(2).mean().sqrt()


def _mixed_norm(tensor_tuple):
    if len(tensor_tuple) == 0:
        return 0.
    return max([_rms_norm(tensor) for tensor in tensor_tuple])


class Problem:
    pass


def _combine_event_functions(event_fn, t0, y0):
    with torch.no_grad():
        initial_signs = torch.sign(event_fn(t0, y0))

    def combined_event_fn(t, y):
        c = event_fn(t, y)
        return torch.min(c * initial_signs)
    return combined_event_fn


def _check_timelike(name, timelike, can_grad, values=None):
    assert isinstance(timelike, torch.Tensor), '{} must be a torch.Tensor'.format(name)
    if not torch.is_floating_point(timelike):
        raise TypeError('`{}` must be a floating point Tensor but is a {}'.format(name, timelike.type()))
    assert timelike.ndimension() == 1, "{} must be one dimensional".format(name)
    if not can_grad:
        assert not timelike.requires_grad, "{} cannot require gradient".format(name)
    v = timelike if values is None else values
    diff = v[1:] > v[:-1]
    assert diff.all() or (~diff).all(), '{} must be strictly increasing or decreasing'.format(name)


def _tol_vector(name, tol, layout, shape, device):
    if isinstance(tol, torch.Tensor):
        if tol.ndim == 0:
            return float(tol), None
        if layout is None:
            return None, tol.detach().to(device=device, dtype=torch.float64).expand(shape).reshape(-1).contiguous()
    else:
        try:
            iter(tol)
        except TypeError:
            return float(tol), None
    assert layout is not None, "tupled {} needs a tuple y0".format(name)
    tol = tuple(tol)
    assert len(tol) == len(layout.shapes), \
        "If using tupled {} it must have the same length as the tuple y0".format(name)
    vec = torch.ones(layout.n, dtype=torch.float64, device=device)
    for tol_, o, l, shp in zip(tol, layout.offsets, layout.lens, layout.shapes):
        v = torch.as_tensor(tol_).to(device)
        vec[o:o + l] = v.expand(shp).reshape(-1).to(torch.float64)
    return None, vec


def normalise(func, y0, t, rtol, atol, method, options, event_fn, adjoint=False):
    if event_fn is not None:
        if len(t) != 2:
            raise ValueError(f"We require len(t) == 2 when in event handling mode, but got len(t)={len(t)}.")
        event_fn = _combine_event_functions(event_fn, t[0], y0)
    p = Problem()
    p.original_func = func
    p.is_tuple = not isinstance(y0, torch.Tensor)
    if p.is_tuple:
        assert isinstance(y0, tuple), 'y0 must be either a torch.Tensor or a tuple'
        p.layout = Layout([y_.shape for y_ in y0], y0[0].dtype)
        p.device = y0[0].device
        p.dtype = y0[0].dtype
    else:
        p.layout = None
        p.device = y0.device
        p.dtype = y0.dtype
    options = {} if options is None else options.copy()
    if method is None:
        method = 'dopri5'
    if method not in REFERENCE_METHODS:
        raise ValueError('Invalid method "{}". Must be one of {}'.format(
            method, '{"' + '", "'.join(REFERENCE_METHODS) + '"}.'))
    if method not in ADAPTIVE_METHODS + FIXED_METHODS + tuple(ADAMS_METHODS):
        raise NotImplementedError('method "{}" is not part of the B200 hot path; implemented: {}'.format(
            method, ADAPTIVE_METHODS + FIXED_METHODS + tuple(ADAMS_METHODS)))
    p.method, p.options = method, options
    if p.device.type != "cuda":
        raise _lib.TdqError("torchdiffeq_b200 runs on CUDA devices only (got %s); there is no CPU path" % p.device)
    _lib.load()

    t_cpu = t.detach().to("cpu") if isinstance(t, torch.Tensor) else t
    _check_timelike('t', t, True, values=t_cpu)
    p.t_reversed = bool(len(t_cpu) > 1 and t_cpu[0] > t_cpu[1])
    p.t_sign = -1.0 if p.t_reversed else 1.0
    p.t_cpu = -t_cpu if p.t_reversed else t_cpu
    if p.t_reversed:
        for name in ("step_t", "jump_t"):
            if isinstance(options.get(name), torch.Tensor):
                options[name] = -options[name]
        if "grid_constructor" in options:
            _gc = options["grid_constructor"]
            options["grid_constructor"] = lambda func, y0, t: -_gc(func, y0, -t)
    assert (p.t_cpu[1:] > p.t_cpu[:-1]).all(), 't must be strictly increasing or decreasing'

    if torch.is_tensor(rtol):
        assert not rtol.requires_grad, "rtol cannot require gradient"
    if torch.is_tensor(atol):
        assert not atol.requires_grad, "atol cannot require gradient"
    if t.device != p.device:
        warnings.warn("t is not on the same device as y0. Coercing to y0.device.")

    shape_ = None if p.is_tuple else y0.shape
    p.rtol, p.rtol_vec = _tol_vector('rtol', rtol, p.layout, shape_, p.device)
    p.atol, p.atol_vec = _tol_vector('atol', atol, p.layout, shape_, p.device)
    if (p.rtol_vec is None) != (p.atol_vec is None):
        if p.rtol_vec is None:
            p.rtol_vec = torch.full_like(p.atol_vec, p.rtol)
        else:
            p.atol_vec = torch.full_like(p.rtol_vec, p.atol)

    p.callbacks = {}
    for name in _CALLBACK_NAMES:
        cb = getattr(func, name, None)
        if cb is not None:
            p.callbacks[name] = cb
    valid = set(_CALLBACK_NAMES) if method in ADAPTIVE_METHODS else {"callback_step"}
    invalid = set(p.callbacks) - valid
    if invalid:
        warnings.warn("Solver '{}' does not support callbacks {}".format(method, invalid))
        for name in invalid:
            del p.callbacks[name]
    if p.callbacks:
        layout, sign = p.layout, p.t_sign
        def _wrap(cb):
            def _cb(t0, y0_flat, dt):
                y_ = layout.views(y0_flat) if layout is not None else y0_flat.view(p.shape)
                return cb(t0 * sign, y_, dt)
            return _cb
        p.callbacks = {k: _wrap(v) for k, v in p.callbacks.items()}

    if p.is_tuple:
        p.shape = None
        p.y0_flat = p.layout.flatten([y_.detach() for y_ in y0])
        p.n = p.layout.n
        layout = p.layout
        def fn(t_, y_flat):
            f = func(t_, layout.views(y_flat))
            return tuple(f)
        p.fn = fn
        p.pieces = (list(layout.offsets), list(layout.lens), [1.0] * len(layout.lens))
        p.segs = list(zip(layout.offsets, layout.lens))
    else:
        p.shape = y0.shape
        p.y0_flat = y0.detach().reshape(-1)
        p.n = p.y0_flat.numel()
        shape = p.shape
        p.fn = lambda t_, y_flat: func(t_, y_flat.view(shape))
        p.pieces = None
        p.segs = None

    p.event_fn = None
    if event_fn is not None:
        unflat = (lambda yf: p.layout.views(yf)) if p.is_tuple else (lambda yf: yf.view(p.shape))
        sign_ = p.t_sign
        p.event_fn = lambda t_, y_flat: event_fn(t_ * sign_, unflat(y_flat))

    p.norm_fn = None
    p.q_view = None
    user_norm = options.get("norm", None)
    if user_norm is not None and user_norm is not _rms_norm and not (p.is_tuple and user_norm is _mixed_norm):
        p.norm_fn = user_norm
        if p.is_tuple:
            p.q_view = lambda q: layout.views(q)
        else:
            p.q_view = lambda q: q.view(shape)
    return p


def _warn_unused(solver_name, options, known):
    unused = {k: v for k, v in options.items() if k not in known and k not in _OUR_OPTIONS}
    if unused:
        warnings.warn('{}: Unexpected arguments {}'.format(solver_name, unused))


def _resolve_graph(graph, func):
    if graph == "auto" and not isinstance(func, torch.nn.Module):
        return False
    return graph


def _make_adaptive_engine(p, method, rtol, atol, rtol_vec, atol_vec, options, fn=None, n=None, segs=None,
                          pieces=None, norm_fn=None, q_view=None, callbacks=None, solver_name=None,
                          keep_interp=False, replicated=(), post_fn=None):
    o = options
    _warn_unused(solver_name or method, o, _ADAPTIVE_OPTIONS)
    graph = _resolve_graph(o.get("graph", "auto"), getattr(p, "original_func", None))
    if o.get("dtype", torch.float64) != torch.float64:
        raise NotImplementedError("time dtype other than float64 (options['dtype']) is not implemented")
    def _tvals(v):
        v = torch.as_tensor(v, dtype=torch.float64).to("cpu")
        return torch.sort(v[v >= p.t_cpu[0].double()]).values
    step_t, jump_t = o.get("step_t"), o.get("jump_t")
    st = _tvals(step_t) if step_t is not None else torch.tensor([], dtype=torch.float64)
    jt = _tvals(jump_t) if jump_t is not None else torch.tensor([], dtype=torch.float64)
    if (torch.cat([st, jt]).unique(return_counts=True)[1] > 1).any():
        raise ValueError("`step_t` and `jump_t` must not have any repeated elements between them.")
    step_t = st.to(p.device) if step_t is not None else None
    jump_t = jt.to(p.device) if jump_t is not None else None
    reduce_fn, n_global, seg_counts_global, agree_fn, exchange = None, None, None, None, None
    pg = o.get("process_group")
    if pg is not None:
        from .dist import make_agree, make_reduce
        if norm_fn is not None:
            raise NotImplementedError("a custom norm callable cannot be evaluated on a batch-sharded state "
                                      "(SURVEY.md section 8(e): replicas only); use the default norm or 'seminorm'")
        reduce_fn, n_global, seg_counts_global = make_reduce(pg, segs if segs is not None else
                                                             [(0, n if n is not None else p.n)], p.device,
                                                             replicated=replicated)
        agree_fn = make_agree(pg)
        if o.get("exchange", "peer") == "peer" and norm_fn is None:
            try:
                from .dist import PeerExchange
                n_seg_ = len(segs) if segs is not None else 1
                if n_seg_ > _lib.TDQ_MAX_SEGS:
                    raise _lib.TdqError("more than %d norm segments" % _lib.TDQ_MAX_SEGS)
                exchange = PeerExchange(pg, p.device)
            except Exception as e:
                warnings.warn("torchdiffeq_b200: NVLink peer exchange unavailable (%s: %s); using the process "
                              "group's all-reduce" % (type(e).__name__, e))
    eng = AdaptiveEngine(
        fn if fn is not None else p.fn, n if n is not None else p.n, p.dtype, p.device, method,
        rtol=rtol, atol=atol, rtol_vec=rtol_vec, atol_vec=atol_vec,
        segs=segs, t_sign=p.t_sign, pieces=pieces,
        min_step=o.get("min_step", 0), max_step=o.get("max_step", float("inf")),
        first_step=o.get("first_step"), step_t=step_t, jump_t=jump_t,
        safety=o.get("safety", 0.9), ifactor=o.get("ifactor", 10.0), dfactor=o.get("dfactor", 0.2),
        max_num_steps=o.get("max_num_steps", 2 ** 31 - 1),
        norm_fn=norm_fn, q_view=q_view, graph=graph, run_ahead=o.get("run_ahead", 2),
        reduce_fn=reduce_fn, n_global=n_global, seg_counts_global=seg_counts_global, agree_fn=agree_fn,
        exchange=exchange, callbacks=callbacks, keep_interp=keep_interp, device_loop=o.get("device_loop", "auto"),
        post_fn=post_fn)
    if fn is None and not p.is_tuple and o.get("fused_linear", True):
        from .fields import fusable
        w = fusable(getattr(p, "original_func", None), tuple(p.shape), p.dtype, p.device, eng.lib)
        if w is not None:
            eng.set_linear(w, whole_attempt=o.get("fused_attempt", True), fused_controller=o.get("fused_controller", True))
    return eng


_ENGINE_CACHE = collections.OrderedDict()
_BACKWARD_CACHE = collections.OrderedDict()
_CACHE_MAX = {"forward": 4, "backward": 4}


def clear_cache():
    _ENGINE_CACHE.clear()
    _BACKWARD_CACHE.clear()


def set_cache_size(forward=4, backward=4):
    _CACHE_MAX["forward"], _CACHE_MAX["backward"] = int(forward), int(backward)
    for which, c in (("forward", _ENGINE_CACHE), ("backward", _BACKWARD_CACHE)):
        while len(c) > _CACHE_MAX[which]:
            c.popitem(last=False)


def _tensor_sig(x):
    return (x.data_ptr(), tuple(x.shape), x.dtype, x.requires_grad)


_PLAIN = (int, float, bool, str, type(None), complex)


def _attr_sig(name, v):
    if isinstance(v, torch.Tensor):
        return (name,) + _tensor_sig(v)
    if isinstance(v, _PLAIN):
        return (name, v)
    if isinstance(v, (list, tuple)):
        items = tuple(_attr_sig(i, x) for i, x in enumerate(v) if isinstance(x, (torch.Tensor,) + _PLAIN))
        return (name, type(v).__name__, len(v), items)
    if isinstance(v, dict):
        items = tuple(_attr_sig(str(k), x) for k, x in v.items() if isinstance(x, (torch.Tensor,) + _PLAIN))
        return (name, "dict", len(v), items)
    return None


_SKIP_ATTRS = {"_parameters", "_buffers", "_modules", "_non_persistent_buffers_set", "_backward_hooks",
               "_backward_pre_hooks", "_forward_hooks", "_forward_pre_hooks", "_forward_hooks_with_kwargs",
               "_forward_pre_hooks_with_kwargs", "_forward_hooks_always_called", "_state_dict_hooks",
               "_state_dict_pre_hooks", "_load_state_dict_pre_hooks", "_load_state_dict_post_hooks",
               "_is_full_backward_hook", "_compiled_call_impl", "training"}


def _func_signature(func, explicit=False):
    if isinstance(func, torch.nn.Module):
        sig = [id(func)]
        for name, m in func.named_modules():
            sig.append((name, type(m).__name__, m.training))
            sig.extend((name,) + _tensor_sig(q) for q in m.parameters(recurse=False))
            sig.extend((name,) + _tensor_sig(b) for b in m.buffers(recurse=False))
            for k, v in vars(m).items():
                if k in _SKIP_ATTRS:
                    continue
                a = _attr_sig(k, v)
                if a is not None:
                    sig.append((name,) + a)
        return tuple(sig)
    if explicit:
        return (id(func),)
    return None


def _cache_key(p, extra=()):
    o = p.options
    if o.get("cache", True) is False or p.callbacks or p.norm_fn is not None or p.rtol_vec is not None:
        return None
    fsig = _func_signature(p.original_func, explicit=o.get("cache", None) is True)
    if fsig is None:
        return None
    items = []
    for k, v in sorted(o.items()):
        if k == "process_group":
            v = id(v)
        elif isinstance(v, torch.Tensor) or callable(v):
            return None
        items.append((k, v))
    shapes = tuple(tuple(s_) for s_ in p.layout.shapes) if p.is_tuple else tuple(p.shape)
    try:
        key = (fsig, p.method, p.dtype, str(p.device), p.is_tuple, shapes, p.rtol, p.atol,
               p.t_sign, tuple(items), torch.is_autocast_enabled(), extra)
        hash(key)
    except TypeError:
        return None
    return key


def _cache_get(key, which="forward"):
    c = _ENGINE_CACHE if which == "forward" else _BACKWARD_CACHE
    if key is None or key not in c:
        return None
    c.move_to_end(key)
    return c[key]


def _cache_put(key, value, which="forward"):
    if key is None:
        return
    c = _ENGINE_CACHE if which == "forward" else _BACKWARD_CACHE
    c[key] = value
    while len(c) > _CACHE_MAX[which]:
        c.popitem(last=False)


def _cache_drop(key, which="forward"):
    c = _ENGINE_CACHE if which == "forward" else _BACKWARD_CACHE
    if key is not None:
        c.pop(key, None)


_LAST_STATS = {}


def last_stats():
    return dict(_LAST_STATS)


def _solve(p):
    if p.method in ADAPTIVE_METHODS:
        key = _cache_key(p)
        hit = _cache_get(key)
        if hit is not None:
            eng = hit[0]
        else:
            eng = _make_adaptive_engine(p, p.method, p.rtol, p.atol, p.rtol_vec, p.atol_vec, p.options,
                                        segs=p.segs, pieces=p.pieces, norm_fn=p.norm_fn, q_view=p.q_view,
                                        callbacks=p.callbacks)
            _cache_put(key, (eng, p.original_func))
        t64 = p.t_cpu.to(torch.float64).to(p.device)
        try:
            sol = eng.solve(p.y0_flat, t64, t_start=float(p.t_cpu[0]))
        except BaseException:
            _cache_drop(key)
            raise
        if key is not None:
            sol = sol.clone()
        return sol, eng
    o = p.options
    y0_view = p.layout.views(p.y0_flat) if p.is_tuple else p.y0_flat.view(p.shape)
    grid = fixed_grid(p.method, o, p.original_func, y0_view, p.t_cpu)
    eng = _fixed_engine(p)
    sol = eng.solve(p.y0_flat, grid, p.t_cpu)
    return sol, eng


def _cubic_or_linear(interp):
    if interp not in ("linear", "cubic"):
        raise ValueError(f"Unknown interpolation method {interp}")
    return interp


def fixed_event_solve(eng, y0_flat, t0, step_size, event_fn, atol):
    return eng.solve_until_event(y0_flat, t0, step_size, event_fn, atol)


_FIXED_NAMES = {"euler": "Euler", "midpoint": "Midpoint", "heun2": "Heun2", "heun3": "Heun3", "rk4": "RK4",
                "explicit_adams": "AdamsBashforth", "implicit_adams": "AdamsBashforthMoulton",
                "fixed_adams": "AdamsBashforthMoulton"}


def _fixed_engine(p, graph=None, interp=None):
    o = p.options
    interp = _cubic_or_linear(o.get("interp", "linear")) if interp is None else interp
    if p.method in ADAMS_METHODS:
        from ._adams import AdamsEngine
        if p.rtol is None or p.atol is None:
            raise NotImplementedError("per-element tolerances are not implemented for the Adams methods")
        return AdamsEngine(p.fn, p.n, p.dtype, p.device, implicit=ADAMS_METHODS[p.method], rtol=p.rtol, atol=p.atol,
                           max_iters=o.get("max_iters", 4), max_order=o.get("max_order", 12), t_sign=p.t_sign,
                           perturb=o.get("perturb", False), callbacks=p.callbacks, pieces=p.pieces, interp=interp)
    g = _resolve_graph(o.get("graph", "auto"), p.original_func) if graph is None else graph
    return FixedGridEngine(p.fn, p.n, p.dtype, p.device, method=p.method, t_sign=p.t_sign,
                           perturb=o.get("perturb", False), graph=g, callbacks=p.callbacks, pieces=p.pieces, interp=interp)


def fixed_grid(method, o, func, y0_view, t_cpu, keep_graph=False):
    _warn_unused(_FIXED_NAMES[method], o, _ADAMS_OPTIONS if method in ADAMS_METHODS else _FIXED_OPTIONS)
    step_size, gc = o.get("step_size"), o.get("grid_constructor")
    if step_size is None:
        grid_constructor = gc if gc is not None else (lambda f, y0, t: t)
    else:
        if gc is not None:
            raise ValueError("step_size and grid_constructor are mutually exclusive arguments.")
        grid_constructor = grid_from_step_size(step_size)
    _cubic_or_linear(o.get("interp", "linear"))
    grid = grid_constructor(func, y0_view, t_cpu)
    grid = grid.to("cpu") if keep_graph else grid.detach().to("cpu")
    assert grid[0] == t_cpu[0] and grid[-1] == t_cpu[-1]
    return grid


def _solve_event(p):
    if p.method in FIXED_METHODS or p.method in ADAMS_METHODS:
        o = p.options
        _warn_unused(_FIXED_NAMES[p.method], o, _ADAMS_OPTIONS if p.method in ADAMS_METHODS else _FIXED_OPTIONS)
        if o.get("step_size") is None:
            raise AssertionError("Event handling for fixed step solvers currently requires `step_size` to be provided "
                                 "in options.")
        if o.get("grid_constructor") is not None:
            raise ValueError("step_size and grid_constructor are mutually exclusive arguments.")
        eng = _fixed_engine(p, graph=False)
        tol = p.atol if p.atol is not None else float(p.atol_vec.min())
        event_t, y_event = fixed_event_solve(eng, p.y0_flat, p.t_cpu[0], o["step_size"], p.event_fn, tol)
        sol = torch.stack([p.y0_flat.to(p.dtype), y_event], dim=0)
        return float(event_t) * p.t_sign, sol, eng
    eng = _make_adaptive_engine(p, p.method, p.rtol, p.atol, p.rtol_vec, p.atol_vec,
                                dict(p.options, run_ahead=0, graph=False), segs=p.segs, pieces=p.pieces,
                                norm_fn=p.norm_fn, q_view=p.q_view, callbacks=p.callbacks, keep_interp=True)
    tol = p.atol if p.atol is not None else float(p.atol_vec.min())
    event_t, y_event = eng.solve_until_event(p.y0_flat, float(p.t_cpu[0]), p.event_fn, tol)
    sol = torch.stack([p.y0_flat.to(p.dtype), y_event], dim=0)
    return event_t * p.t_sign, sol, eng


def _unflatten(p, sol):
    if p.is_tuple:
        return p.layout.views(sol, (sol.shape[0],))
    return sol.view(sol.shape[0], *p.shape)


class _ImplicitFnGradientRerouting(torch.autograd.Function):

    @staticmethod
    def forward(ctx, func, event_fn, event_t, state_t):
        ctx.func, ctx.event_fn = func, event_fn
        ctx.save_for_backward(event_t, state_t)
        return event_t.detach(), state_t.detach()

    @staticmethod
    def backward(ctx, grad_t, grad_state):
        func, event_fn = ctx.func, ctx.event_fn
        event_t, state_t = ctx.saved_tensors
        event_t = event_t.detach().clone().requires_grad_(True)
        state_t = state_t.detach().clone().requires_grad_(True)
        f_val = func(event_t, state_t)
        with torch.enable_grad():
            c, (par_dt, dstate) = torch.autograd.functional.vjp(event_fn, (event_t, state_t))
        dcdt = par_dt + torch.sum(dstate * f_val)
        grad_t = grad_t + torch.sum(grad_state * f_val)
        dstate = dstate * (-grad_t / (dcdt + 1e-12)).reshape_as(c)
        return None, None, None, grad_state + dstate


def odeint_event(func, y0, t0, *, event_fn, reverse_time=False, odeint_interface=None, **kwargs):
    if odeint_interface is None:
        odeint_interface = odeint
    if reverse_time:
        t = torch.cat([t0.reshape(-1), t0.reshape(-1).detach() - 1.0])
    else:
        t = torch.cat([t0.reshape(-1), t0.reshape(-1).detach() + 1.0])
    event_t, solution = odeint_interface(func, y0, t, event_fn=event_fn, **kwargs)
    p = normalise(func, y0, t, 0.0, 0.0, kwargs.get("method"), None, event_fn)
    sign_ = p.t_sign
    flat_func = lambda t_, y_flat: _as_flat(p, p.fn(t_ * sign_, y_flat)) * sign_
    if p.is_tuple:
        state_t = p.layout.flatten([s_[-1] for s_ in solution])
    else:
        state_t = solution[-1].reshape(-1)
    if reverse_time:
        event_t = -event_t
    event_t, state_t = _ImplicitFnGradientRerouting.apply(flat_func, p.event_fn, event_t, state_t)
    if reverse_time:
        event_t = -event_t
    if p.is_tuple:
        pieces = p.layout.views(state_t)
        solution = tuple(torch.cat([s_[:-1], s_t[None]], dim=0) for s_, s_t in zip(solution, pieces))
    else:
        solution = torch.cat([solution[:-1], state_t.view(p.shape)[None]], dim=0)
    return event_t, solution


def _as_flat(p, f):
    if isinstance(f, tuple):
        return p.layout.flatten(list(f))
    return f.reshape(-1)


def odeint_dense(func, y0, t0, t1, *, rtol=1e-7, atol=1e-9, method=None, options=None):
    import bisect
    import ctypes as C
    from ._engine import _stream
    assert torch.is_tensor(y0)
    t0_, t1_ = torch.as_tensor(t0), torch.as_tensor(t1)
    t = torch.stack([t0_.reshape(()), t1_.reshape(()).to(t0_)]).to(t0_)
    p = normalise(func, y0, t, rtol, atol, method, options, None)
    assert p.method == "dopri5"
    with torch.no_grad(), on_solver_stream(p.device) as ss:
        eng = _make_adaptive_engine(p, p.method, p.rtol, p.atol, p.rtol_vec, p.atol_vec,
                                    dict(p.options, run_ahead=0, graph=False), segs=p.segs, pieces=p.pieces,
                                    norm_fn=p.norm_fn, q_view=p.q_view, callbacks=p.callbacks, keep_interp=True)
        t64 = p.t_cpu.to(torch.float64).to(p.device)
        _, times, coeffs = eng.solve_dense(p.y0_flat, t64)
    lib, dc, n, sign_, shape, dtype, dev = eng.lib, eng.dt_code, p.n, p.t_sign, p.shape, p.dtype, p.device
    ptrs = [_lib.ptr_array([c.data_ptr() for c in cs]) for cs in coeffs]

    def dense_output_fn(t_eval):
        te = float(t_eval) * sign_
        idx = bisect.bisect_right(times, te)
        idx = min(max(idx, 1), len(times) - 1)
        lo, hi = times[idx - 1], times[idx]
        assert lo <= te <= hi, 'invalid interpolation, fails `t0 <= t <= t1`: {}, {}, {}'.format(lo, te, hi)
        out = torch.empty(n, dtype=dtype, device=dev)
        with on_solver_stream(dev) as ss2:
            _lib.check(lib.tdq_poly_eval(dc, ptrs[idx - 1], (te - lo) / (hi - lo), out.data_ptr(), n, _stream()))
            ss2.publish(out)
        return out.view(shape)
    dense_output_fn._keep = (coeffs, ptrs)
    return dense_output_fn


def _odeint_backprop(p, func, y0, t, params, _stats):
    from .backprop import _BackpropFunction, adaptive_tableau
    if p.is_tuple:
        y0_flat = p.layout.flatten(list(y0))
    else:
        y0_flat = y0.reshape(-1)
    holder = {}

    def run():
        if p.method in ADAPTIVE_METHODS:
            eng = _make_adaptive_engine(p, p.method, p.rtol, p.atol, p.rtol_vec, p.atol_vec,
                                        dict(p.options, run_ahead=0, graph=False), segs=p.segs, pieces=p.pieces,
                                        norm_fn=p.norm_fn, q_view=p.q_view, callbacks=p.callbacks)
            t64 = p.t_cpu.to(torch.float64).to(p.device)
            sol, tape = eng.solve_taped(p.y0_flat, t64, t_start=float(p.t_cpu[0]))
            holder["eng"] = eng
            return sol.clone(), {"kind": "adaptive", "tape": tape, "tab": adaptive_tableau(p.method)}
        o = p.options
        if p.method in ADAMS_METHODS:
            raise NotImplementedError("gradients of the discrete solve are implemented for the explicit Runge-Kutta "
                                      "methods; use odeint_adjoint with the Adams methods")
        if o.get("interp", "linear") != "linear":
            raise NotImplementedError("gradients through interp='cubic' are not implemented (use the default linear "
                                      "interpolation, or odeint_adjoint)")
        y0_view = p.layout.views(p.y0_flat) if p.is_tuple else p.y0_flat.view(p.shape)
        with torch.enable_grad():
            t_req = p.t_cpu.detach().clone().requires_grad_(True)
            grid_req = fixed_grid(p.method, o, p.original_func, y0_view, t_req, keep_graph=True)
        grid = grid_req.detach()
        eng = FixedGridEngine(p.fn, p.n, p.dtype, p.device, method=p.method, t_sign=p.t_sign,
                              perturb=o.get("perturb", False), graph=False, callbacks=p.callbacks, pieces=p.pieces)
        sol, tape = eng.solve_taped(p.y0_flat, grid, p.t_cpu)
        holder["eng"] = eng
        return sol, {"kind": "fixed", "tape": tape, "grid": grid, "grid_req": grid_req, "t_req": t_req}
    with on_solver_stream(p.device) as ss:
        sol = _BackpropFunction.apply(p, run, t, y0_flat, *params)
        ss.publish(sol)
    eng = holder.get("eng")
    if eng is not None:
        _LAST_STATS.clear()
        _LAST_STATS.update(nfe=eng.nfe, launches=getattr(eng, "launches", 0), attempts=getattr(eng, "n_attempts", None),
                           n_accept=getattr(eng, "n_accept", None), n_reject=getattr(eng, "n_reject", None),
                       fused_linear=getattr(eng, "linear", None) is not None,
                       fused_attempt=bool((getattr(eng, "linear", None) or {}).get("whole")))
        if _stats is not None:
            _stats.update(_LAST_STATS)
    return _unflatten(p, sol)


def odeint(func, y0, t, *, rtol=1e-7, atol=1e-9, method=None, options=None, event_fn=None, _stats=None):
    p = normalise(func, y0, t, rtol, atol, method, options, event_fn)
    if torch.is_grad_enabled():
        from .backprop import discover_params
        y_req = any(y_.requires_grad for y_ in y0) if p.is_tuple else y0.requires_grad
        params = discover_params(func)
        if y_req or t.requires_grad or params:
            if p.event_fn is not None:
                if isinstance(func, torch.nn.Module):
                    warnings.warn("torchdiffeq_b200.odeint(event_fn=...): gradients are computed with the adjoint method",
                                  stacklevel=2)
                    from .adjoint import odeint_adjoint
                    return odeint_adjoint(func, y0, t, rtol=rtol, atol=atol, method=method, options=options,
                                          event_fn=event_fn)
                raise NotImplementedError("gradients through odeint(event_fn=...) need an nn.Module func (they are "
                                          "computed by odeint_adjoint)")
            return _odeint_backprop(p, func, y0, t, params, _stats)
    with torch.no_grad(), on_solver_stream(p.device) as ss:
        if p.event_fn is not None:
            event_t, sol, eng = _solve_event(p)
            ss.publish(sol)
            return torch.tensor(event_t, dtype=t.dtype, device=t.device), _unflatten(p, sol)
        sol, eng = _solve(p)
        ss.publish(sol)
    _LAST_STATS.clear()
    _LAST_STATS.update(nfe=eng.nfe, launches=getattr(eng, "launches", 0), attempts=getattr(eng, "n_attempts", None),
                       n_accept=getattr(eng, "n_accept", None), n_reject=getattr(eng, "n_reject", None),
                       fused_linear=getattr(eng, "linear", None) is not None,
                       fused_attempt=bool((getattr(eng, "linear", None) or {}).get("whole")))
    if _stats is not None:
        _stats["nfe"] = eng.nfe
        _stats["launches"] = _stats.get("launches", 0) + getattr(eng, "launches", 0)
        _stats["attempts"] = getattr(eng, "n_attempts", None)
        _stats["n_accept"], _stats["n_reject"] = getattr(eng, "n_accept", None), getattr(eng, "n_reject", None)
        _stats["fused_linear"], _stats["fused_attempt"] = _LAST_STATS["fused_linear"], _LAST_STATS["fused_attempt"]
    return _unflatten(p, sol)
```

Baseline: 8.033 million.

## Add cooperative persistent kernel running multiple dopri5 attempts with in-kernel grid sync

Adds a cooperative-launch kernel for the fused linear field that loops over several step attempts inside one launch. It synchronises the grid on the device for the error-norm reduction and the controller step, instead of relaunching per attempt through the graph conditional loop. The aim is to remove per-attempt launch overhead, repeated TMEM/weight setup and graph-iteration cost. In exchange it adds grid-wide barrier waits, a grid timeout failure mode, and a dependency on cooperative launch residency limits.

```diff
diff --git a/include/tdq.h b/include/tdq.h
--- a/include/tdq.h
+++ b/include/tdq.h
@@ -29,7 +29,8 @@
     TDQ_RUN_DT_UNDERFLOW = 1,
     TDQ_RUN_NONFINITE = 2,
     TDQ_RUN_MAX_STEPS = 3,
-    TDQ_RUN_EXCHANGE_TIMEOUT = 4
+    TDQ_RUN_EXCHANGE_TIMEOUT = 4,
+    TDQ_RUN_GRID_TIMEOUT = 5
 } tdq_run_status;
 
 typedef struct {
@@ -73,6 +74,7 @@
     volatile double next_t0, next_dt;
     volatile int32_t on_jump_t;
     volatile int32_t par;
+    volatile int64_t n_solve_launches;
 } tdq_mailbox;
 
 int tdq_abi_version(void);
@@ -169,6 +171,11 @@
                        const void *y0, const void *k0, const void *planes, int32_t width, size_t n, double *partials,
                        double *norm_out, const int64_t *seg_counts_dev, int32_t store_always, void *stream);
 
+int tdq_linear_solve_supported(const tdq_tableau *tab, int32_t dtype, int32_t width);
+int tdq_linear_solve(void *ctrl_dev, const tdq_tableau *tab, int32_t dtype, void *const *k_out, void *y1_out, void *err_out,
+                     const void *planes, int32_t width, size_t n, double *partials, double *norm_out,
+                     const int64_t *seg_counts_dev, void *stream);
+
 int tdq_fixed_emit_cubic(int32_t dtype, const void *y0, const void *y1, const void *f0, const void *f1, void *solution,
                          const int32_t *out_idx_dev, const void *coef_dev, int32_t rec_lo, int32_t rec_hi, size_t n,
                          void *stream);
diff --git a/torchdiffeq_b200/_engine.py b/torchdiffeq_b200/_engine.py
--- a/torchdiffeq_b200/_engine.py
+++ b/torchdiffeq_b200/_engine.py
@@ -218,6 +218,9 @@
         self._loop = None
         self._loop_handle = 0
         self._loop_failed = False
+        self._loop_fused = False
+        self._solve_kernel = False
+        self.ran_fused_loop = False
         self._always_copy = False
         self.linear = None
         self.capture_in_solve = True
@@ -261,7 +264,7 @@
             self.post_fn(buf)
         return buf
 
-    def set_linear(self, weight, whole_attempt=True, fused_controller=True):
+    def set_linear(self, weight, whole_attempt=True, fused_controller=True, fused_loop=True):
         width, S = int(weight.shape[0]), self.S
         if self.pieces is not None or self.post_fn is not None or self.n % width:
             return False
@@ -275,8 +278,10 @@
         planes = torch.empty(int(self.lib.tdq_linear_weights_bytes(width)), dtype=torch.uint8, device=self.device)
         whole = bool(whole_attempt) and bool(self.lib.tdq_linear_attempt_supported(C.byref(self.tab), self.dt_code, width))
         fold = (whole and self.norm_table is None and self.n_seg == 1 and self.rtol_vec is None and self.norm_fn is None)
+        loop = (bool(fused_loop) and fold and bool(fused_controller) and self.n > 0
+                and bool(self.lib.tdq_linear_solve_supported(C.byref(self.tab), self.dt_code, width)))
         self.linear = dict(weight=weight, width=width, planes=planes, whole=whole, fold=fold, ctrl=bool(fused_controller),
-                           k=[torch.zeros(self.n, dtype=self.dtype, device=self.device) for _ in range(S)])
+                           loop=loop, k=[torch.zeros(self.n, dtype=self.dtype, device=self.device) for _ in range(S)])
         self._drop_graph()
         return True
 
@@ -304,7 +309,7 @@
                 self.lib.tdq_loop_destroy(self._loop)
             except Exception:
                 pass
-        self._loop, self._loop_handle = None, 0
+        self._loop, self._loop_handle, self._loop_fused = None, 0, False
         self._graph, self._graph_keep = None, None
 
     def _launch(self, rc):
@@ -354,6 +359,12 @@
                 k[i + 1] = L["k"][i].data_ptr()
             folded = L["fold"]
             with_ctrl = folded and L["ctrl"] and (self.reduce_fn is None or self.exchange is not None)
+            if self._solve_kernel:
+                self._launch(lib.tdq_linear_solve(ctrl, tab, dc, _lib.ptr_array(k), self.y1.data_ptr(), self.errp.data_ptr(),
+                                                  L["planes"].data_ptr(), L["width"], self.n, self.partials.data_ptr(),
+                                                  self.norm_out.data_ptr(), self.seg_counts.data_ptr(), st))
+                self.nfe += S
+                return k, _lib.ptr_array(k), keep
             self._launch(lib.tdq_linear_attempt(ctrl, tab, dc, _lib.ptr_array(k), self.y1.data_ptr(), self.errp.data_ptr(),
                                                 None, None, L["planes"].data_ptr(), L["width"], self.n,
                                                 self.partials.data_ptr() if folded else None,
@@ -441,6 +452,8 @@
             raise SolverFailure("underflow in dt {}".format(mb.next_dt))
         if s == _lib.RUN_NONFINITE:
             raise SolverFailure("non-finite values in state `y`: {}".format(self.y0w))
+        if s == _lib.RUN_GRID_TIMEOUT:
+            raise _lib.TdqError("a block of the multi-attempt kernel waited more than 20 s for the rest of the grid")
         if s == _lib.RUN_EXCHANGE_TIMEOUT:
             raise _lib.TdqError("a peer rank did not deliver its norm partials within 10 s (sharded solve)")
         if s == _lib.RUN_MAX_STEPS:
@@ -449,6 +462,11 @@
 
     def _lockstep_mode(self):
         return bool(self.callbacks) or self.run_ahead == 0
+
+    def _fused_loop_eligible(self):
+        L = self.linear
+        return bool(L is not None and L["whole"] and L["loop"] and (self.reduce_fn is None or self.exchange is not None)
+                    and not self.callbacks and self.agree_fn is None and self.norm_fn is None)
 
     def _use_loop(self):
         return (self._loop is not None and not self._lockstep_mode() and self.agree_fn is None
@@ -489,6 +507,7 @@
         lib = self.lib
         self.nfe_total += self.nfe
         self.nfe, self.launches = 0, 0
+        self.ran_fused_loop = False
         n_out = int(t64.numel())
         self.t_out = t64.contiguous()
         if getattr(self, "solution", None) is None or self.solution.shape[0] != n_out:
@@ -714,7 +733,8 @@
         mb = self.mbox_host.contents
         ran = int(mb.seq) - first
         self.nfe += self.S * ran
-        self.launches += self._graph_launches * ran
+        self.launches += self._graph_launches * (int(mb.n_solve_launches) if self._loop_fused else ran)
+        self.ran_fused_loop = self._loop_fused
         self._raise_if_failed(mb)
 
     def _warm_attempt(self):
@@ -726,17 +746,24 @@
             try:
                 want_loop = (self.device_loop in (True, "auto") and not self._loop_failed and self.agree_fn is None
                              and self.norm_fn is None)
+                fused = want_loop and self._fused_loop_eligible()
                 g = torch.cuda.CUDAGraph(keep_graph=True) if want_loop else torch.cuda.CUDAGraph()
                 nfe, launches = self.nfe, self.launches
+                self._solve_kernel = fused
                 try:
                     with torch.cuda.graph(g, stream=solver_stream(self.device)):
                         keep = self._attempt()
                 finally:
+                    self._solve_kernel = False
                     self._graph_launches = self.launches - launches
                     self.nfe, self.launches = nfe, launches
                 self._graph, self._graph_keep = g, keep
                 if want_loop:
                     self._make_loop(g)
+                    self._loop_fused = fused and self._loop is not None
+                    if fused and self._loop is None:
+                        self._graph, self._graph_keep = None, None
+                        return self._capture()
                 return
             except Exception as e:
                 last = e
diff --git a/torchdiffeq_b200/_lib.py b/torchdiffeq_b200/_lib.py
--- a/torchdiffeq_b200/_lib.py
+++ b/torchdiffeq_b200/_lib.py
@@ -8,7 +8,7 @@
 TDQ_MAX_K = TDQ_MAX_STAGES + 1
 TDQ_MAX_SEGS = 64
 TDQ_F32, TDQ_F64 = 0, 1
-RUN_OK, RUN_DT_UNDERFLOW, RUN_NONFINITE, RUN_MAX_STEPS, RUN_EXCHANGE_TIMEOUT = 0, 1, 2, 3, 4
+RUN_OK, RUN_DT_UNDERFLOW, RUN_NONFINITE, RUN_MAX_STEPS, RUN_EXCHANGE_TIMEOUT, RUN_GRID_TIMEOUT = 0, 1, 2, 3, 4, 5
 TDQ_MAX_RANKS = 16
 ABI_VERSION = 2
 
@@ -51,6 +51,7 @@
         ("ratio", C.c_double), ("att_t0", C.c_double), ("att_dt", C.c_double),
         ("next_t0", C.c_double), ("next_dt", C.c_double),
         ("on_jump_t", C.c_int32), ("par", C.c_int32),
+        ("n_solve_launches", C.c_int64),
     ]
 
 
@@ -112,6 +113,8 @@
     "tdq_linear_stage": (C.c_int, [_vp, _ptab, _i32, _i32, _vp, _vp, _vp, _vp, _pp, _vp, _i32, _sz, _vp]),
     "tdq_linear_attempt_supported": (C.c_int, [_ptab, _i32, _i32]),
     "tdq_linear_attempt": (C.c_int, [_vp, _ptab, _i32, _pp, _vp, _vp, _vp, _vp, _vp, _i32, _sz, _vp, _vp, _vp, _i32, _vp]),
+    "tdq_linear_solve_supported": (C.c_int, [_ptab, _i32, _i32]),
+    "tdq_linear_solve": (C.c_int, [_vp, _ptab, _i32, _pp, _vp, _vp, _vp, _i32, _sz, _vp, _vp, _vp, _vp]),
     "tdq_fixed_emit_cubic": (C.c_int, [_i32, _vp, _vp, _vp, _vp, _vp, _vp, _vp, _i32, _i32, _sz, _vp]),
     "tdq_pack_segments": (C.c_int, [_i32, _vp, _pp, _pi64, _pi64, _pdbl, _i32, _vp]),
     "tdq_xchg_create": (C.c_int, [_pp, C.POINTER(IpcHandle)]),
diff --git a/torchdiffeq_b200/csrc/tdq_attempt.cu b/torchdiffeq_b200/csrc/tdq_attempt.cu
--- a/torchdiffeq_b200/csrc/tdq_attempt.cu
+++ b/torchdiffeq_b200/csrc/tdq_attempt.cu
@@ -66,51 +66,82 @@
     return n;
 }
 
-template <int S, unsigned long long RM, unsigned EM, int G, int RT, bool CTRL, int ACCS>
-__global__ void __launch_bounds__(G * 128 * (16 / RT), 1)
-k_linear_attempt(TdqCtrl *c, const float *y0, const float *k0, AttOut out, const uint32_t *__restrict__ wt,
-                 double *partials, double *norm_out, const int64_t *seg_counts, int store_always, size_t n_rows_sz) {
+template <int G>
+struct SmemView {
+    uint32_t bar0;
+    uint32_t *tmem_slot;
+    int *s_flag, *s_exit;
+    float *s_cr, *s_ce;
+    double *s_red;
+    __device__ __forceinline__ explicit SmemView(uint8_t *smem) {
+        uint8_t *aux = smem + G * (AT_STAGE + AT_Y0);
+        bar0 = smem_u32(aux);
+        tmem_slot = reinterpret_cast<uint32_t *>(aux + 32);
+        s_flag = reinterpret_cast<int *>(aux + 40);
+        s_exit = reinterpret_cast<int *>(aux + 44);
+        s_cr = reinterpret_cast<float *>(aux + 64);
+        s_ce = s_cr + AT_MAX_S * 8;
+        s_red = reinterpret_cast<double *>(aux + 512);
+    }
+};
+template <int S, int G>
+__device__ __forceinline__ void load_coefs(const TdqCtrl *c, const SmemView<G> &v, int tid) {
+    if (tid >= 64 && tid < 64 + AT_MAX_S * 8) {
+        const int i = (tid - 64) >> 3, m = (tid - 64) & 7;
+        v.s_cr[i * 8 + m] = (i < S) ? (float)c->coef[i][m] : 0.f;
+        if (i == 0) v.s_ce[m] = (float)c->ecoef[m];
+    }
+}
+template <typename T> __device__ __forceinline__ T tdq_opaque(T x);
+template <> __device__ __forceinline__ uint32_t tdq_opaque<uint32_t>(uint32_t x) {
+    asm volatile("mov.b32 %0, %0;" : "+r"(x));
+    return x;
+}
+template <> __device__ __forceinline__ uint64_t tdq_opaque<uint64_t>(uint64_t x) {
+    asm volatile("mov.b64 %0, %0;" : "+l"(x));
+    return x;
+}
+
+template <int S, unsigned long long RM, unsigned EM, int G, int RT, bool CTRL, int ACCS, bool LOOP>
+__device__ __forceinline__ void linear_attempts(TdqCtrl *c, const float *y0_arg, const float *k0_arg, const AttOut &out,
+                                                const uint32_t *__restrict__ wt, double *partials, double *norm_out,
+                                                const int64_t *seg_counts, int store_always, size_t n_rows_sz) {
+    static_assert(!LOOP || CTRL, "the multi-attempt kernel runs the controller step");
+    constexpr int AT_GROUPS = G, HN = AT_ROWS / RT, WPG = 4 * HN, AT_THREADS = G * 128 * HN;
     if (c->halt) {
-        if (CTRL && blockIdx.x == 0) tdq_ctrl_dev::controller_block<float, G * 128 * (16 / RT)>(c, norm_out, seg_counts, 1, nullptr);
+        if (CTRL && blockIdx.x == 0) {
+            if (LOOP) {
+                if (threadIdx.x == 0) c->n_solve_launches += 1;
+                __syncthreads();
+            }
+            tdq_ctrl_dev::controller_block<float, AT_THREADS>(c, norm_out, seg_counts, 1, nullptr);
+        }
         return;
     }
     extern __shared__ uint8_t smem_raw[];
     uint8_t *smem = reinterpret_cast<uint8_t *>((reinterpret_cast<uintptr_t>(smem_raw) + 1023) & ~(uintptr_t)1023);
-    constexpr int AT_GROUPS = G, HN = AT_ROWS / RT, WPG = 4 * HN, AT_THREADS = G * 128 * HN;
-    uint8_t *aux = smem + G * (AT_STAGE + AT_Y0);
-    uint64_t *bars = reinterpret_cast<uint64_t *>(aux);
-    uint32_t *tmem_slot = reinterpret_cast<uint32_t *>(aux + 32);
-    int *s_flag = reinterpret_cast<int *>(aux + 40);
-    float *s_cr = reinterpret_cast<float *>(aux + 64);
-    float *s_ce = s_cr + AT_MAX_S * 8;
-    double *s_red = reinterpret_cast<double *>(aux + 512);
-    const int tid = threadIdx.x, lane = tid & 31;
-    const int warp = __shfl_sync(0xffffffffu, tid >> 5, 0);
-    const int n_rows = (int)n_rows_sz;
-    const uint32_t bar0 = smem_u32(bars);
-
-    if (warp == 0) {
-        asm volatile("tcgen05.alloc.cta_group::1.sync.aligned.shared::cta.b32 [%0], %1;" :: "r"(smem_u32(tmem_slot)), "n"(AT_TMEM_COLS) : "memory");
-        asm volatile("tcgen05.relinquish_alloc_permit.cta_group::1.sync.aligned;" ::: "memory");
-    }
-    if (tid == 32) {
-#pragma unroll
-        for (int g = 0; g < AT_GROUPS; ++g) mbar_init(bar0 + 8 * g, 1);
-        asm volatile("fence.mbarrier_init.release.cluster;" ::: "memory");
-    }
-    if (tid >= 64 && tid < 64 + AT_MAX_S * 8) {
-        const int i = (tid - 64) >> 3, m = (tid - 64) & 7;
-        s_cr[i * 8 + m] = (i < S) ? (float)c->coef[i][m] : 0.f;
-        if (i == 0) s_ce[m] = (float)c->ecoef[m];
-    }
-    fence_before();
-    __syncthreads();
-    fence_after();
-    const uint32_t tmem = __shfl_sync(0xffffffffu, *tmem_slot, 0);
-
-    const int g = warp / WPG, wl = warp % WPG, e = wl & 3, h = wl >> 2, f = e * 32 + lane;
-    const uint32_t lane_base = tmem + ((uint32_t)(e * 32) << 16);
+    uint32_t tmem;
     {
+        const SmemView<G> v(smem);
+        const int tid = threadIdx.x, lane = tid & 31;
+        const int warp = __shfl_sync(0xffffffffu, tid >> 5, 0);
+        if (warp == 0) {
+            asm volatile("tcgen05.alloc.cta_group::1.sync.aligned.shared::cta.b32 [%0], %1;" :: "r"(smem_u32(v.tmem_slot)), "n"(AT_TMEM_COLS) : "memory");
+            asm volatile("tcgen05.relinquish_alloc_permit.cta_group::1.sync.aligned;" ::: "memory");
+        }
+        if (tid == 32) {
+#pragma unroll
+            for (int g = 0; g < AT_GROUPS; ++g) mbar_init(v.bar0 + 8 * g, 1);
+            asm volatile("fence.mbarrier_init.release.cluster;" ::: "memory");
+        }
+        if (LOOP && blockIdx.x == 0 && tid == 0) c->n_solve_launches += 1;
+        load_coefs<S, G>(c, v, tid);
+        fence_before();
+        __syncthreads();
+        fence_after();
+        tmem = __shfl_sync(0xffffffffu, *v.tmem_slot, 0);
+        const int f = (warp & 3) * 32 + lane;
+        const uint32_t lane_base = tmem + ((uint32_t)((warp & 3) * 32) << 16);
 #pragma unroll 1
         for (int ch = warp >> 2; ch < 6; ch += AT_THREADS / 128) {
             const int pl = ch >> 1, c0 = (ch & 1) * 32;
@@ -118,327 +149,410 @@
             const uint4 *src = reinterpret_cast<const uint4 *>(wt + ((size_t)pl * LD + f) * 64 + c0);
 #pragma unroll
             for (int j = 0; j < 8; ++j) {
-                const uint4 v = src[j];
-                r[4 * j] = v.x; r[4 * j + 1] = v.y; r[4 * j + 2] = v.z; r[4 * j + 3] = v.w;
+                const uint4 w4 = src[j];
+                r[4 * j] = w4.x; r[4 * j + 1] = w4.y; r[4 * j + 2] = w4.z; r[4 * j + 3] = w4.w;
             }
             tmem_st32(lane_base + AT_COL_W + pl * 64 + c0, r);
         }
         asm volatile("tcgen05.wait::st.sync.aligned;" ::: "memory");
-    }
-    fence_before();
-    __syncthreads();
-    fence_after();
-
-    if (y0 == nullptr) y0 = reinterpret_cast<const float *>(c->y0_cur);
-    if (k0 == nullptr) k0 = reinterpret_cast<const float *>(c->k0_cur);
-    y0 = tdq_detach(y0, n_rows_sz);
-    k0 = tdq_detach(k0, n_rows_sz);
-    const bool fold = partials != nullptr;
-    float *ycand = nullptr, *kcand = nullptr;
-    if (fold && c->ybuf[0] != nullptr) {
-        ycand = tdq_detach(reinterpret_cast<float *>(c->ybuf[c->par ^ 1]), n_rows_sz);
-        kcand = tdq_detach(reinterpret_cast<float *>(c->kbuf[c->par ^ 1]), n_rows_sz);
-    }
-    bool store = store_always != 0 || c->always_fit != 0;
-    if (!store) {
-        const int cur = c->out_cursor;
-        store = cur < c->n_out && !(c->t_out[cur] > c->att_t1);
-    }
-    const float rtolT = (float)c->rtol, atolT = (float)c->atol;
+        fence_before();
+        __syncthreads();
+        fence_after();
+    }
+    const bool fold = LOOP || partials != nullptr;
     constexpr int EK = popc_below(EM, S);
-    const float ecS = s_ce[EK];
-
-    uint8_t *stage = smem + g * AT_STAGE;
-    const uint32_t sy0 = smem_u32(smem + AT_GROUPS * AT_STAGE + g * AT_Y0) + (uint32_t)(h * RT * LD + f) * 4;
-    const uint32_t stage_u32 = smem_u32(stage);
-    const uint32_t bar = bar0 + 8 * g;
     constexpr int ACOLS = 32 * ACCS;
-    const uint32_t acc0 = tmem + g * ACOLS;
     uint32_t phase = 0;
-    const uint32_t st_f = stage_u32 + (uint32_t)f * 16 + (uint32_t)(h * (RT / 8)) * AT_SBO;
-
-    const int tiles = (n_rows + AT_ROWS - 1) / AT_ROWS;
-    const int workers = (int)gridDim.x * AT_GROUPS;
-    double acc = 0.0;
-    int nbad = 0;
-    const uint32_t zero32 = (uint32_t)(n_rows_sz >> 63);
-
-    constexpr int KEEP = S < 4 ? S : 4;
-    constexpr int NACC = S - KEEP;
-    auto row_mask = [](int i) -> unsigned { return (unsigned)((RM >> (8 * i)) & 0xffull); };
-    auto do_tile = [&](auto full_tag, const int t) {
-        constexpr bool FULL = decltype(full_tag)::value;
-        const int row0 = t * AT_ROWS;
-        const int rows_here = FULL ? RT : n_rows - row0 - h * RT;
-        const size_t base = (size_t)(row0 + h * RT) * LD + f;
-        float K[KEEP][RT];
-        float A[NACC > 0 ? NACC : 1][RT];
-        float AE[RT], PRE[RT], KN[RT], Y1[RT];
-        {
-            float Y0[RT];
-#pragma unroll
-            for (int r = 0; r < RT; ++r) {
-                Y0[r] = 0.f;
-                KN[r] = 0.f;
-                if (FULL || r < rows_here) {
-                    Y0[r] = __ldcs(y0 + base + (size_t)r * LD);
-                    KN[r] = __ldcs(k0 + base + (size_t)r * LD);
-                }
-            }
-#pragma unroll
-            for (int r = 0; r < RT; ++r) sts_f32(sy0 + r * LD * 4, Y0[r]);
-        }
-#pragma unroll
-        for (int i = 0; i < S; ++i) {
-            const unsigned mask = row_mask(i);
-            const bool last = i == S - 1;
-            const bool has_prefix = (mask & ((1u << i) - 1u)) != 0u, has_new = ((mask >> i) & 1u) != 0u;
-            const float c_new = has_new ? s_cr[i * 8 + popc_below(mask, i)] : 0.f;
-            if (i < KEEP) {
-#pragma unroll
-                for (int r = 0; r < RT; ++r) K[i < KEEP ? i : 0][r] = KN[r];
-            }
-#pragma unroll
-            for (int r8 = 0; r8 < RT; r8 += 8) {
-                uint32_t H[4], M[4], L[4];
-#pragma unroll
-                for (int r = r8; r < r8 + 8; r += 2) {
-                    float yv[2];
-#pragma unroll
-                    for (int q = 0; q < 2; ++q) {
-                        const float pre = i < KEEP ? PRE[r + q] : A[i >= KEEP ? i - KEEP : 0][r + q];
-                        float sum;
-                        if (has_prefix && has_new) sum = pre + KN[r + q] * c_new;
-                        else if (has_prefix) sum = pre;
-                        else sum = KN[r + q] * c_new;
-                        yv[q] = lds_f32(sy0 + (r + q) * LD * 4) + sum;
-                        if (last) Y1[r + q] = yv[q];
-                    }
-                    split2(yv[0], yv[1], H[(r - r8) >> 1], M[(r - r8) >> 1], L[(r - r8) >> 1]);
-                }
-                sts_v4(st_f + (r8 >> 3) * AT_SBO, H[0], H[1], H[2], H[3]);
-                sts_v4(st_f + AT_PLANE + (r8 >> 3) * AT_SBO, M[0], M[1], M[2], M[3]);
-                sts_v4(st_f + 2 * AT_PLANE + (r8 >> 3) * AT_SBO, L[0], L[1], L[2], L[3]);
-            }
-            fence_async_smem();
-            fence_before();
-            asm volatile("bar.sync %0, %1;" :: "r"(g + 1), "n"(WPG * 32) : "memory");
-            if (wl == g % 4 && elect_one()) {
-                fence_after();
-                constexpr int NPROD = 6;
-                constexpr int PW[NPROD] = {1, 2, 0, 1, 0, 0}, PY[NPROD] = {1, 0, 2, 0, 1, 0};
-#pragma unroll
-                for (int p = 0; p < NPROD; ++p) {
-#pragma unroll
-                    for (int ks = 0; ks < 8; ++ks) {
-                        const uint32_t dcol = acc0 + (ks % ACCS) * 32 + (p == NPROD - 1 ? 0 : 16);
-                        mma_ts(dcol, tmem + AT_COL_W + PW[p] * 64 + ks * 8, make_desc_mn(stage_u32 + PY[p] * AT_PLANE + ks * 2 * AT_LBO), IDESC16,
-                               (p == 0 || p == NPROD - 1) && ks < ACCS ? 0u : 1u);
-                    }
-                }
-                mma_commit(bar);
-            }
-            __syncwarp();
-            uint32_t dep = 0;
-            if (i + 1 < KEEP && i + 1 < S) {
-                const unsigned mn = row_mask(i + 1);
-                bool first = true;
-#pragma unroll
-                for (int j = 0; j <= i; ++j) {
-                    if ((mn >> j) & 1u) {
-                        const float cj = s_cr[(i + 1) * 8 + popc_below(mn, j)];
-#pragma unroll
-                        for (int r = 0; r < RT; ++r) {
-                            const float p = K[j < KEEP ? j : 0][r] * cj;
-                            PRE[r] = first ? p : PRE[r] + p;
-                        }
-                        first = false;
-                    }
-                }
-                if (!first) dep |= dep16(PRE, zero32);
-            }
-            if (i == KEEP - 1) {
+    int tid_carry = threadIdx.x;
+
+#pragma unroll 1
+    for (;;) {
+        if (LOOP) {
+            tid_carry = (int)tdq_opaque((uint32_t)tid_carry);
+            smem = reinterpret_cast<uint8_t *>(tdq_opaque((uint64_t)smem));
+            tmem = tdq_opaque(tmem);
+        }
+        const SmemView<G> v(smem);
+        const int tid = tid_carry, lane = tid & 31;
+        const int warp = __shfl_sync(0xffffffffu, tid >> 5, 0);
+        const int n_rows = (int)n_rows_sz;
+        int *s_flag = v.s_flag, *s_exit = v.s_exit;
+        const float *s_cr = v.s_cr, *s_ce = v.s_ce;
+        double *s_red = v.s_red;
+        const int g = warp / WPG, wl = warp % WPG, e = wl & 3, h = wl >> 2, f = e * 32 + lane;
+        const uint32_t lane_base = tmem + ((uint32_t)(e * 32) << 16);
+        const float rtolT = (float)c->rtol, atolT = (float)c->atol;
+        uint8_t *stage = smem + g * AT_STAGE;
+        const uint32_t sy0 = smem_u32(smem + AT_GROUPS * AT_STAGE + g * AT_Y0) + (uint32_t)(h * RT * LD + f) * 4;
+        const uint32_t stage_u32 = smem_u32(stage);
+        const uint32_t bar = v.bar0 + 8 * g;
+        const uint32_t acc0 = tmem + g * ACOLS;
+        const uint32_t st_f = stage_u32 + (uint32_t)f * 16 + (uint32_t)(h * (RT / 8)) * AT_SBO;
+        const int tiles = (n_rows + AT_ROWS - 1) / AT_ROWS;
+        const int workers = (int)gridDim.x * AT_GROUPS;
+        const uint32_t zero32 = (uint32_t)(n_rows_sz >> 63);
+
+        const float *y0 = y0_arg != nullptr ? y0_arg : reinterpret_cast<const float *>(c->y0_cur);
+        const float *k0 = k0_arg != nullptr ? k0_arg : reinterpret_cast<const float *>(c->k0_cur);
+        y0 = tdq_detach(y0, n_rows_sz);
+        k0 = tdq_detach(k0, n_rows_sz);
+        float *ycand = nullptr, *kcand = nullptr;
+        if (fold && c->ybuf[0] != nullptr) {
+            ycand = tdq_detach(reinterpret_cast<float *>(c->ybuf[c->par ^ 1]), n_rows_sz);
+            kcand = tdq_detach(reinterpret_cast<float *>(c->kbuf[c->par ^ 1]), n_rows_sz);
+        }
+        bool store = store_always != 0 || c->always_fit != 0;
+        if (!store) {
+            const int cur = c->out_cursor;
+            store = cur < c->n_out && !(c->t_out[cur] > c->att_t1);
+        }
+        const float ecS = s_ce[EK];
+        double acc = 0.0;
+        int nbad = 0;
+
+        constexpr int KEEP = S < 4 ? S : 4;
+        constexpr int NACC = S - KEEP;
+        auto row_mask = [](int i) -> unsigned { return (unsigned)((RM >> (8 * i)) & 0xffull); };
+        auto do_tile = [&](auto full_tag, const int t) {
+            constexpr bool FULL = decltype(full_tag)::value;
+            const int row0 = t * AT_ROWS;
+            const int rows_here = FULL ? RT : n_rows - row0 - h * RT;
+            const size_t base = (size_t)(row0 + h * RT) * LD + f;
+            float K[KEEP][RT];
+            float A[NACC > 0 ? NACC : 1][RT];
+            float AE[RT], PRE[RT], KN[RT], Y1[RT];
+            {
+                float Y0[RT];
 #pragma unroll
                 for (int r = 0; r < RT; ++r) {
-#pragma unroll
-                    for (int qrow = KEEP; qrow < S; ++qrow) {
-                        const unsigned mq = row_mask(qrow);
-                        float a_ = 0.f;
+                    Y0[r] = 0.f;
+                    KN[r] = 0.f;
+                    if (FULL || r < rows_here) {
+                        Y0[r] = __ldcs(y0 + base + (size_t)r * LD);
+                        KN[r] = __ldcs(k0 + base + (size_t)r * LD);
+                    }
+                }
+#pragma unroll
+                for (int r = 0; r < RT; ++r) sts_f32(sy0 + r * LD * 4, Y0[r]);
+            }
+#pragma unroll
+            for (int i = 0; i < S; ++i) {
+                const unsigned mask = row_mask(i);
+                const bool last = i == S - 1;
+                const bool has_prefix = (mask & ((1u << i) - 1u)) != 0u, has_new = ((mask >> i) & 1u) != 0u;
+                const float c_new = has_new ? s_cr[i * 8 + popc_below(mask, i)] : 0.f;
+                if (i < KEEP) {
+#pragma unroll
+                    for (int r = 0; r < RT; ++r) K[i < KEEP ? i : 0][r] = KN[r];
+                }
+#pragma unroll
+                for (int r8 = 0; r8 < RT; r8 += 8) {
+                    uint32_t H[4], M[4], L[4];
+#pragma unroll
+                    for (int r = r8; r < r8 + 8; r += 2) {
+                        float yv[2];
+#pragma unroll
+                        for (int q = 0; q < 2; ++q) {
+                            const float pre = i < KEEP ? PRE[r + q] : A[i >= KEEP ? i - KEEP : 0][r + q];
+                            float sum;
+                            if (has_prefix && has_new) sum = pre + KN[r + q] * c_new;
+                            else if (has_prefix) sum = pre;
+                            else sum = KN[r + q] * c_new;
+                            yv[q] = lds_f32(sy0 + (r + q) * LD * 4) + sum;
+                            if (last) Y1[r + q] = yv[q];
+                        }
+                        split2(yv[0], yv[1], H[(r - r8) >> 1], M[(r - r8) >> 1], L[(r - r8) >> 1]);
+                    }
+                    sts_v4(st_f + (r8 >> 3) * AT_SBO, H[0], H[1], H[2], H[3]);
+                    sts_v4(st_f + AT_PLANE + (r8 >> 3) * AT_SBO, M[0], M[1], M[2], M[3]);
+                    sts_v4(st_f + 2 * AT_PLANE + (r8 >> 3) * AT_SBO, L[0], L[1], L[2], L[3]);
+                }
+                fence_async_smem();
+                fence_before();
+                asm volatile("bar.sync %0, %1;" :: "r"(g + 1), "n"(WPG * 32) : "memory");
+                if (wl == g % 4 && elect_one()) {
+                    fence_after();
+                    constexpr int NPROD = 6;
+                    constexpr int PW[NPROD] = {1, 2, 0, 1, 0, 0}, PY[NPROD] = {1, 0, 2, 0, 1, 0};
+#pragma unroll
+                    for (int p = 0; p < NPROD; ++p) {
+#pragma unroll
+                        for (int ks = 0; ks < 8; ++ks) {
+                            const uint32_t dcol = acc0 + (ks % ACCS) * 32 + (p == NPROD - 1 ? 0 : 16);
+                            mma_ts(dcol, tmem + AT_COL_W + PW[p] * 64 + ks * 8, make_desc_mn(stage_u32 + PY[p] * AT_PLANE + ks * 2 * AT_LBO), IDESC16,
+                                   (p == 0 || p == NPROD - 1) && ks < ACCS ? 0u : 1u);
+                        }
+                    }
+                    mma_commit(bar);
+                }
+                __syncwarp();
+                uint32_t dep = 0;
+                if (i + 1 < KEEP && i + 1 < S) {
+                    const unsigned mn = row_mask(i + 1);
+                    bool first = true;
+#pragma unroll
+                    for (int j = 0; j <= i; ++j) {
+                        if ((mn >> j) & 1u) {
+                            const float cj = s_cr[(i + 1) * 8 + popc_below(mn, j)];
+#pragma unroll
+                            for (int r = 0; r < RT; ++r) {
+                                const float p = K[j < KEEP ? j : 0][r] * cj;
+                                PRE[r] = first ? p : PRE[r] + p;
+                            }
+                            first = false;
+                        }
+                    }
+                    if (!first) dep |= dep16(PRE, zero32);
+                }
+                if (i == KEEP - 1) {
+#pragma unroll
+                    for (int r = 0; r < RT; ++r) {
+#pragma unroll
+                        for (int qrow = KEEP; qrow < S; ++qrow) {
+                            const unsigned mq = row_mask(qrow);
+                            float a_ = 0.f;
+                            bool first = true;
+#pragma unroll
+                            for (int j = 0; j <= i; ++j) {
+                                if ((mq >> j) & 1u) {
+                                    const float p = K[j < KEEP ? j : 0][r] * s_cr[qrow * 8 + popc_below(mq, j)];
+                                    a_ = first ? p : a_ + p;
+                                    first = false;
+                                }
+                            }
+                            A[qrow - KEEP][r] = a_;
+                        }
+                        float e_ = 0.f;
                         bool first = true;
 #pragma unroll
                         for (int j = 0; j <= i; ++j) {
-                            if ((mq >> j) & 1u) {
-                                const float p = K[j < KEEP ? j : 0][r] * s_cr[qrow * 8 + popc_below(mq, j)];
-                                a_ = first ? p : a_ + p;
+                            if ((EM >> j) & 1u) {
+                                const float p = K[j < KEEP ? j : 0][r] * s_ce[popc_below(EM, j)];
+                                e_ = first ? p : e_ + p;
                                 first = false;
                             }
                         }
-                        A[qrow - KEEP][r] = a_;
-                    }
-                    float e_ = 0.f;
-                    bool first = true;
-#pragma unroll
-                    for (int j = 0; j <= i; ++j) {
-                        if ((EM >> j) & 1u) {
-                            const float p = K[j < KEEP ? j : 0][r] * s_ce[popc_below(EM, j)];
-                            e_ = first ? p : e_ + p;
-                            first = false;
-                        }
-                    }
-                    AE[r] = e_;
-                }
-#pragma unroll
-                for (int qrow = KEEP; qrow < S; ++qrow) dep |= dep16(A[qrow - KEEP], zero32);
-                dep |= dep16(AE, zero32);
-            }
-            if (i >= KEEP) {
-#pragma unroll
-                for (int qrow = i + 1; qrow < S; ++qrow) {
-                    const unsigned mq = row_mask(qrow);
-                    if ((mq >> i) & 1u) {
-                        const float cj = s_cr[qrow * 8 + popc_below(mq, i)];
-                        const bool started = (mq & ((1u << i) - 1u)) != 0u;
+                        AE[r] = e_;
+                    }
+#pragma unroll
+                    for (int qrow = KEEP; qrow < S; ++qrow) dep |= dep16(A[qrow - KEEP], zero32);
+                    dep |= dep16(AE, zero32);
+                }
+                if (i >= KEEP) {
+#pragma unroll
+                    for (int qrow = i + 1; qrow < S; ++qrow) {
+                        const unsigned mq = row_mask(qrow);
+                        if ((mq >> i) & 1u) {
+                            const float cj = s_cr[qrow * 8 + popc_below(mq, i)];
+                            const bool started = (mq & ((1u << i) - 1u)) != 0u;
+#pragma unroll
+                            for (int r = 0; r < RT; ++r) {
+                                const float p = KN[r] * cj;
+                                A[qrow - KEEP][r] = started ? A[qrow - KEEP][r] + p : p;
+                            }
+                        }
+                    }
+                    if ((EM >> i) & 1u) {
+                        const float cj = s_ce[popc_below(EM, i)];
+                        const bool started = (EM & ((1u << i) - 1u)) != 0u;
 #pragma unroll
                         for (int r = 0; r < RT; ++r) {
                             const float p = KN[r] * cj;
-                            A[qrow - KEEP][r] = started ? A[qrow - KEEP][r] + p : p;
-                        }
-                    }
-                }
-                if ((EM >> i) & 1u) {
-                    const float cj = s_ce[popc_below(EM, i)];
-                    const bool started = (EM & ((1u << i) - 1u)) != 0u;
+                            AE[r] = started ? AE[r] + p : p;
+                        }
+                    }
+#pragma unroll
+                    for (int qrow = i + 1; qrow < S; ++qrow) dep |= dep16(A[qrow - KEEP], zero32);
+                    dep |= dep16(AE, zero32);
+                }
+                if (last) {
 #pragma unroll
                     for (int r = 0; r < RT; ++r) {
-                        const float p = KN[r] * cj;
-                        AE[r] = started ? AE[r] + p : p;
-                    }
-                }
-#pragma unroll
-                for (int qrow = i + 1; qrow < S; ++qrow) dep |= dep16(A[qrow - KEEP], zero32);
-                dep |= dep16(AE, zero32);
-            }
-            if (last) {
-#pragma unroll
-                for (int r = 0; r < RT; ++r) {
-                    const float y1v = Y1[r];
-                    if (FULL || r < rows_here) {
-                        if (!isfinite(y1v)) nbad += 1;
-                        const size_t o = base + (size_t)r * LD;
-                        if (ycand) ycand[o] = y1v;
-                        if (store) {
-                            out.y1[o] = y1v;
-                            out.err[o] = AE[r];
-                        }
-                    }
-                    Y1[r] = Ar<float>::add(atolT, Ar<float>::mul(rtolT, Ar<float>::max_nan(fabsf(lds_f32(sy0 + r * LD * 4)), fabsf(y1v))));
-                }
-                dep |= dep16(Y1, zero32);
-            }
-            mbar_wait(bar + dep, phase);
-            phase ^= 1u;
+                        const float y1v = Y1[r];
+                        if (FULL || r < rows_here) {
+                            if (!isfinite(y1v)) nbad += 1;
+                            const size_t o = base + (size_t)r * LD;
+                            if (ycand) ycand[o] = y1v;
+                            if (store) {
+                                out.y1[o] = y1v;
+                                out.err[o] = AE[r];
+                            }
+                        }
+                        Y1[r] = Ar<float>::add(atolT, Ar<float>::mul(rtolT, Ar<float>::max_nan(fabsf(lds_f32(sy0 + r * LD * 4)), fabsf(y1v))));
+                    }
+                    dep |= dep16(Y1, zero32);
+                }
+                mbar_wait(bar + dep, phase);
+                phase ^= 1u;
+                fence_after();
+                {
+                    uint32_t tq[RT];
+#pragma unroll
+                    for (int a_ = 0; a_ < 2 * ACCS; ++a_) {
+                        const int col = (a_ < ACCS ? a_ * 32 + 16 : (a_ - ACCS) * 32) + h * RT;
+                        tmem_ldn<RT>(lane_base + (uint32_t)(g * ACOLS + col), tq);
+                        asm volatile("tcgen05.wait::ld.sync.aligned;" ::: "memory");
+#pragma unroll
+                        for (int r = 0; r < RT; ++r) KN[r] = a_ == 0 ? __uint_as_float(tq[r]) : KN[r] + __uint_as_float(tq[r]);
+                    }
+                }
+                if (store) {
+#pragma unroll
+                    for (int r = 0; r < RT; ++r)
+                        if (FULL || r < rows_here) out.k[i + 1][base + (size_t)r * LD] = KN[r];
+                }
+                if (last) {
+#pragma unroll
+                    for (int r = 0; r < RT; ++r) {
+                        if (FULL || r < rows_here) {
+                            if (kcand) kcand[base + (size_t)r * LD] = KN[r];
+                            if (fold) {
+                                const float num = Ar<float>::add(AE[r], Ar<float>::mul(KN[r], ecS));
+                                const float q = Ar<float>::div(num, Y1[r]);
+                                acc += (double)Ar<float>::mul(q, q);
+                            }
+                        }
+                    }
+                }
+            }
+        };
+#pragma unroll 1
+        for (int t = g * (int)gridDim.x + (int)blockIdx.x; t < tiles; t += workers) {
+            {
+                const int tn = t + workers, pr = lane & 15;
+                const long long prow = (long long)tn * AT_ROWS + h * RT + pr;
+                if (tn < tiles && pr < RT && prow < (long long)n_rows) {
+                    const float *pp = (lane < 16 ? y0 : k0) + (size_t)prow * LD + e * 32;
+                    asm volatile("prefetch.global.L2 [%0];" :: "l"(pp));
+                }
+            }
+            if (n_rows - t * AT_ROWS >= AT_ROWS) do_tile(std::true_type{}, t);
+            else do_tile(std::false_type{}, t);
+        }
+        const double bad = (double)nbad;
+
+        if (fold) {
+            const double wa = warp_sum(acc), wb = warp_sum(bad);
+            if (lane == 0) {
+                s_red[warp] = wa;
+                s_red[32 + warp] = wb;
+            }
+        }
+        fence_before();
+        __syncthreads();
+        if (!LOOP && warp == 0) {
             fence_after();
-            {
-                uint32_t tq[RT];
-#pragma unroll
-                for (int a_ = 0; a_ < 2 * ACCS; ++a_) {
-                    const int col = (a_ < ACCS ? a_ * 32 + 16 : (a_ - ACCS) * 32) + h * RT;
-                    tmem_ldn<RT>(lane_base + (uint32_t)(g * ACOLS + col), tq);
-                    asm volatile("tcgen05.wait::ld.sync.aligned;" ::: "memory");
-#pragma unroll
-                    for (int r = 0; r < RT; ++r) KN[r] = a_ == 0 ? __uint_as_float(tq[r]) : KN[r] + __uint_as_float(tq[r]);
-                }
-            }
-            if (store) {
-#pragma unroll
-                for (int r = 0; r < RT; ++r)
-                    if (FULL || r < rows_here) out.k[i + 1][base + (size_t)r * LD] = KN[r];
-            }
-            if (last) {
-#pragma unroll
-                for (int r = 0; r < RT; ++r) {
-                    if (FULL || r < rows_here) {
-                        if (kcand) kcand[base + (size_t)r * LD] = KN[r];
-                        if (fold) {
-                            const float num = Ar<float>::add(AE[r], Ar<float>::mul(KN[r], ecS));
-                            const float q = Ar<float>::div(num, Y1[r]);
-                            acc += (double)Ar<float>::mul(q, q);
-                        }
-                    }
-                }
-            }
-        }
-    };
-#pragma unroll 1
-    for (int t = g * (int)gridDim.x + (int)blockIdx.x; t < tiles; t += workers) {
-        {
-            const int tn = t + workers, pr = lane & 15;
-            const long long prow = (long long)tn * AT_ROWS + h * RT + pr;
-            if (tn < tiles && pr < RT && prow < (long long)n_rows) {
-                const float *pp = (lane < 16 ? y0 : k0) + (size_t)prow * LD + e * 32;
-                asm volatile("prefetch.global.L2 [%0];" :: "l"(pp));
-            }
-        }
-        if (n_rows - t * AT_ROWS >= AT_ROWS) do_tile(std::true_type{}, t);
-        else do_tile(std::false_type{}, t);
-    }
-    const double bad = (double)nbad;
-
-    if (fold) {
-        const double wa = warp_sum(acc), wb = warp_sum(bad);
-        if (lane == 0) {
-            s_red[warp] = wa;
-            s_red[32 + warp] = wb;
-        }
-    }
-    fence_before();
-    __syncthreads();
-    if (warp == 0) {
+            asm volatile("tcgen05.dealloc.cta_group::1.sync.aligned.b32 %0, %1;" :: "r"(tmem), "n"(AT_TMEM_COLS) : "memory");
+        }
+        if (!fold) return;
+        const int P = (int)gridDim.x;
+        double *p_sum = partials + 2, *p_bad = p_sum + P;
+        unsigned int *ticket = reinterpret_cast<unsigned int *>(partials);
+        unsigned int *gen = ticket + 2;
+        unsigned int gen0 = 0;
+        if (tid == 0) {
+            double a = 0.0, b = 0.0;
+            for (int w = 0; w < AT_THREADS / 32; ++w) {
+                a += s_red[w];
+                b += s_red[32 + w];
+            }
+            p_sum[blockIdx.x] = a;
+            p_bad[blockIdx.x] = b;
+            if (LOOP) asm volatile("ld.acquire.gpu.global.u32 %0, [%1];" : "=r"(gen0) : "l"(gen) : "memory");
+            __threadfence();
+            const unsigned int tk = atomicAdd(ticket, 1u);
+            *s_flag = (tk == gridDim.x - 1) ? 1 : 0;
+        }
+        __syncthreads();
+        if (!LOOP && !*s_flag) return;
+        if (*s_flag) {
+            __threadfence();
+            if (warp == 0) {
+                double a = 0.0, b = 0.0;
+                for (int i = lane; i < P; i += 32) {
+                    a += __ldcg(&p_sum[i]);
+                    b += __ldcg(&p_bad[i]);
+                }
+                a = warp_sum(a);
+                b = warp_sum(b);
+                if (lane == 0) {
+                    norm_out[0] = a;
+                    norm_out[1] = b;
+                    *ticket = 0;
+                }
+            }
+            if (CTRL) {
+                __threadfence();
+                __syncthreads();
+                tdq_ctrl_dev::controller_block<float, AT_THREADS>(c, norm_out, seg_counts, 1, nullptr, !LOOP);
+            }
+        }
+        if (!LOOP) return;
+
+        __syncthreads();
+        if (tid == 0) {
+            if (*s_flag) {
+                __threadfence();
+                asm volatile("st.release.gpu.global.u32 [%0], %1;" :: "l"(gen), "r"(gen0 + 1u) : "memory");
+            }
+            unsigned int seen = gen0;
+            unsigned long long t_start = 0, now = 0;
+            asm volatile("mov.u64 %0, %%globaltimer;" : "=l"(t_start));
+            do {
+                asm volatile("ld.acquire.gpu.global.u32 %0, [%1];" : "=r"(seen) : "l"(gen) : "memory");
+                if (seen != gen0) break;
+                asm volatile("mov.u64 %0, %%globaltimer;" : "=l"(now));
+            } while (now - t_start < 20000000000ull);
+            volatile TdqCtrl *vc = c;
+            if (seen == gen0) {
+                vc->status = TDQ_RUN_GRID_TIMEOUT;
+                vc->halt = 1;
+                if (vc->mbox) {
+                    vc->mbox->status = TDQ_RUN_GRID_TIMEOUT;
+                    __threadfence_system();
+                }
+            }
+            *s_exit = (vc->halt || vc->fit_now || vc->always_fit) ? 1 : 0;
+        }
+        __syncthreads();
+        if (*s_exit) break;
+        load_coefs<S, G>(c, v, tid);
+        __syncthreads();
+    }
+
+    if ((threadIdx.x >> 5) == 0) {
         fence_after();
         asm volatile("tcgen05.dealloc.cta_group::1.sync.aligned.b32 %0, %1;" :: "r"(tmem), "n"(AT_TMEM_COLS) : "memory");
     }
-    if (!fold) return;
-    const int P = (int)gridDim.x;
-    double *p_sum = partials + 2, *p_bad = p_sum + P;
-    unsigned int *ticket = reinterpret_cast<unsigned int *>(partials);
-    if (tid == 0) {
-        double a = 0.0, b = 0.0;
-        for (int w = 0; w < AT_THREADS / 32; ++w) {
-            a += s_red[w];
-            b += s_red[32 + w];
-        }
-        p_sum[blockIdx.x] = a;
-        p_bad[blockIdx.x] = b;
-        __threadfence();
-        const unsigned int tk = atomicAdd(ticket, 1u);
-        *s_flag = (tk == gridDim.x - 1) ? 1 : 0;
-    }
-    __syncthreads();
-    if (!*s_flag) return;
-    __threadfence();
-    if (warp == 0) {
-        double a = 0.0, b = 0.0;
-        for (int i = lane; i < P; i += 32) {
-            a += __ldcg(&p_sum[i]);
-            b += __ldcg(&p_bad[i]);
-        }
-        a = warp_sum(a);
-        b = warp_sum(b);
-        if (lane == 0) {
-            norm_out[0] = a;
-            norm_out[1] = b;
-            *ticket = 0;
-        }
-    }
-    if (CTRL) {
-        __threadfence();
-        __syncthreads();
-        tdq_ctrl_dev::controller_block<float, AT_THREADS>(c, norm_out, seg_counts, 1, nullptr);
-    }
+    if (blockIdx.x == 0 && threadIdx.x == 0 && c->loop_handle != 0ull)
+        cudaGraphSetConditional((cudaGraphConditionalHandle)c->loop_handle, c->halt ? 0u : 1u);
+}
+
+template <int S, unsigned long long RM, unsigned EM, int G, int RT, bool CTRL, int ACCS>
+__global__ void __launch_bounds__(G * 128 * (16 / RT), 1)
+k_linear_attempt(TdqCtrl *c, const float *y0, const float *k0, AttOut out, const uint32_t *__restrict__ wt,
+                 double *partials, double *norm_out, const int64_t *seg_counts, int store_always, size_t n_rows_sz) {
+    linear_attempts<S, RM, EM, G, RT, CTRL, ACCS, false>(c, y0, k0, out, wt, partials, norm_out, seg_counts, store_always, n_rows_sz);
+}
+
+template <int S, unsigned long long RM, unsigned EM, int G, int RT, int ACCS>
+__global__ void __launch_bounds__(G * 128 * (16 / RT), 1)
+k_linear_solve(TdqCtrl *c, AttOut out, const uint32_t *__restrict__ wt, double *partials, double *norm_out,
+               const int64_t *seg_counts, size_t n_rows_sz) {
+    linear_attempts<S, RM, EM, G, RT, true, ACCS, true>(c, nullptr, nullptr, out, wt, partials, norm_out, seg_counts, 0, n_rows_sz);
 }
 
 constexpr unsigned long long RM_DOPRI5 = 0x01ull | (0x03ull << 8) | (0x07ull << 16) | (0x0full << 24) | (0x1full << 32) | (0x3dull << 40);
 constexpr unsigned long long RM_BOSH3 = 0x01ull | (0x02ull << 8) | (0x07ull << 16);
+
+unsigned attempt_grid(size_t n_rows, int G) {
+    const size_t tiles = (n_rows + AT_ROWS - 1) / AT_ROWS;
+    size_t grid = (tiles + G - 1) / G;
+    const size_t cap = (size_t)tdq_sm_count();
+    if (grid > cap) grid = cap;
+    if (grid == 0) grid = 1;
+    return (unsigned)grid;
+}
 
 template <int S, unsigned long long RM, unsigned EM, int G, int RT, bool CTRL, int ACCS>
 int launch_attempt_g(TdqCtrl *c, const float *y0, const float *k0, const AttOut &out, const uint32_t *wt, double *partials,
@@ -446,22 +560,39 @@
     auto kern = k_linear_attempt<S, RM, EM, G, RT, CTRL, ACCS>;
     constexpr int AT_SMEM = at_smem(G);
     if (cudaFuncSetAttribute(kern, cudaFuncAttributeMaxDynamicSharedMemorySize, AT_SMEM) != cudaSuccess) return -2;
-    const size_t tiles = (n_rows + AT_ROWS - 1) / AT_ROWS;
-    size_t grid = (tiles + G - 1) / G;
-    const size_t cap = (size_t)tdq_sm_count();
-    if (grid > cap) grid = cap;
-    if (grid == 0) grid = 1;
-    kern<<<(unsigned)grid, G * 128 * (AT_ROWS / RT), AT_SMEM, st>>>(c, y0, k0, out, wt, partials, norm_out, seg_counts, store_always, n_rows);
+    const unsigned grid = attempt_grid(n_rows, G);
+    kern<<<grid, G * 128 * (AT_ROWS / RT), AT_SMEM, st>>>(c, y0, k0, out, wt, partials, norm_out, seg_counts, store_always, n_rows);
     return 0;
 }
+
+constexpr int AT_G = 4, AT_RT = 16, AT_ACCS = 1;
 
 template <int S, unsigned long long RM, unsigned EM>
 int launch_attempt(TdqCtrl *c, const float *y0, const float *k0, const AttOut &out, const uint32_t *wt, double *partials,
                    double *norm_out, const int64_t *seg_counts, int store_always, size_t n_rows, cudaStream_t st) {
-#define TDQ_GO(G_, RT_, A_) (seg_counts ? launch_attempt_g<S, RM, EM, G_, RT_, true, A_>(c, y0, k0, out, wt, partials, norm_out, seg_counts, store_always, n_rows, st) \
-                                        : launch_attempt_g<S, RM, EM, G_, RT_, false, A_>(c, y0, k0, out, wt, partials, norm_out, seg_counts, store_always, n_rows, st))
-    return TDQ_GO(4, 16, 1);
-#undef TDQ_GO
+    return seg_counts ? launch_attempt_g<S, RM, EM, AT_G, AT_RT, true, AT_ACCS>(c, y0, k0, out, wt, partials, norm_out, seg_counts, store_always, n_rows, st)
+                      : launch_attempt_g<S, RM, EM, AT_G, AT_RT, false, AT_ACCS>(c, y0, k0, out, wt, partials, norm_out, seg_counts, store_always, n_rows, st);
+}
+
+template <int S, unsigned long long RM, unsigned EM>
+int launch_solve(TdqCtrl *c, const AttOut &out, const uint32_t *wt, double *partials, double *norm_out, const int64_t *seg_counts,
+                 size_t n_rows, cudaStream_t st) {
+    auto kern = k_linear_solve<S, RM, EM, AT_G, AT_RT, AT_ACCS>;
+    constexpr int AT_SMEM = at_smem(AT_G), THREADS = AT_G * 128 * (AT_ROWS / AT_RT);
+    if (cudaFuncSetAttribute(kern, cudaFuncAttributeMaxDynamicSharedMemorySize, AT_SMEM) != cudaSuccess) return -2;
+    int occ = 0;
+    if (cudaOccupancyMaxActiveBlocksPerMultiprocessor(&occ, kern, THREADS, AT_SMEM) != cudaSuccess || occ < 1) return -2;
+    cudaLaunchConfig_t cfg = {};
+    cfg.gridDim = dim3(attempt_grid(n_rows, AT_G));
+    cfg.blockDim = dim3(THREADS);
+    cfg.dynamicSmemBytes = AT_SMEM;
+    cfg.stream = st;
+    cudaLaunchAttribute attr[1];
+    attr[0].id = cudaLaunchAttributeCooperative;
+    attr[0].val.cooperative = 1;
+    cfg.attrs = attr;
+    cfg.numAttrs = 1;
+    return cudaLaunchKernelEx(&cfg, kern, c, out, wt, partials, norm_out, seg_counts, n_rows) == cudaSuccess ? 0 : -3;
 }
 
 bool attempt_masks(const TdqHostShape &hs, unsigned long long *rm, unsigned *em) {
@@ -540,4 +671,51 @@
     return TDQ_OK;
 }
 
-}
+int tdq_linear_solve_supported(const tdq_tableau *tab, int32_t dtype, int32_t width) {
+    if (!tdq_linear_attempt_supported(tab, dtype, width)) return 0;
+    int dev = 0, coop = 0;
+    if (cudaGetDevice(&dev) != cudaSuccess || cudaDeviceGetAttribute(&coop, cudaDevAttrCooperativeLaunch, dev) != cudaSuccess) {
+        cudaGetLastError();
+        return 0;
+    }
+    return coop ? 1 : 0;
+}
+
+int tdq_linear_solve(void *ctrl_dev, const tdq_tableau *tab, int32_t dtype, void *const *k_out, void *y1_out, void *err_out,
+                     const void *planes, int32_t width, size_t n, double *partials, double *norm_out, const int64_t *seg_counts_dev,
+                     void *stream) {
+    TDQ_REQUIRE(ctrl_dev && tab && k_out && y1_out && err_out && planes && partials && norm_out && seg_counts_dev, "null argument");
+    TDQ_REQUIRE(dtype == TDQ_F32 && width == LD, "the fused linear field is float32, width 128");
+    TDQ_REQUIRE(n % (size_t)width == 0 && n > 0, "state size is not a positive multiple of the field width");
+    const size_t n_rows = n / (size_t)width;
+    TDQ_REQUIRE(n_rows < ((size_t)1 << 31) - 64, "too many rows");
+    TdqHostShape hs;
+    tdq_shape_from_tableau(tab, &hs);
+    unsigned long long rm = 0;
+    unsigned em = 0;
+    TDQ_REQUIRE(attempt_masks(hs, &rm, &em), "the whole-attempt kernel takes FSAL tableaus of at most 7 stages");
+    const int S = hs.n_stages;
+    AttOut out;
+    memset(&out, 0, sizeof(out));
+    for (int i = 1; i <= S; ++i) {
+        TDQ_REQUIRE(k_out[i] != nullptr, "missing stage slot");
+        out.k[i] = (float *)k_out[i];
+    }
+    out.y1 = (float *)y1_out;
+    out.err = (float *)err_out;
+    TdqCtrl *c = (TdqCtrl *)ctrl_dev;
+    const uint32_t *wt = (const uint32_t *)planes;
+    cudaStream_t st = (cudaStream_t)stream;
+    int rc = -1;
+    if (S == 6 && rm == RM_DOPRI5 && em == 0x3du)
+        rc = launch_solve<6, RM_DOPRI5, 0x3du>(c, out, wt, partials, norm_out, seg_counts_dev, n_rows, st);
+    else if (S == 3 && rm == RM_BOSH3 && em == 0x07u)
+        rc = launch_solve<3, RM_BOSH3, 0x07u>(c, out, wt, partials, norm_out, seg_counts_dev, n_rows, st);
+    TDQ_REQUIRE(rc != -1, "no whole-attempt kernel for this tableau (tdq_linear_solve_supported)");
+    TDQ_REQUIRE(rc != -2, "launch configuration failed");
+    TDQ_CHECK_CUDA(cudaGetLastError());
+    TDQ_REQUIRE(rc == 0, "cooperative launch failed");
+    return TDQ_OK;
+}
+
+}
diff --git a/torchdiffeq_b200/csrc/tdq_common.cuh b/torchdiffeq_b200/csrc/tdq_common.cuh
--- a/torchdiffeq_b200/csrc/tdq_common.cuh
+++ b/torchdiffeq_b200/csrc/tdq_common.cuh
@@ -25,7 +25,8 @@
     const double *t_out;
     const double *step_t;
     const double *jump_t;
-    int32_t n_jump_t, next_jump_index, on_jump_t, pad_jump;
+    int32_t n_jump_t, next_jump_index, on_jump_t;
+    int32_t n_solve_launches;
     tdq_mailbox *mbox;
     void *xpeer[TDQ_MAX_RANKS];
     unsigned long long xepoch;
diff --git a/torchdiffeq_b200/csrc/tdq_ctrl_dev.cuh b/torchdiffeq_b200/csrc/tdq_ctrl_dev.cuh
--- a/torchdiffeq_b200/csrc/tdq_ctrl_dev.cuh
+++ b/torchdiffeq_b200/csrc/tdq_ctrl_dev.cuh
@@ -150,6 +150,7 @@
     m->next_dt = c.att_dt;
     m->on_jump_t = jumped;
     m->par = c.par;
+    m->n_solve_launches = c.n_solve_launches;
     __threadfence_system();
     m->seq = c.seq;
 }
@@ -248,7 +249,8 @@
 static_assert(sizeof(TdqCtrl) <= 40 * 1024, "control block must fit static shared memory");
 
 template <typename T, int THREADS>
-__device__ void controller_block(TdqCtrl *c, const double *norm_in, const int64_t *cnt, int n_seg, const void *ratio_dev) {
+__device__ void controller_block(TdqCtrl *c, const double *norm_in, const int64_t *cnt, int n_seg, const void *ratio_dev,
+                                 bool set_cond = true) {
     __shared__ __align__(16) unsigned char raw[sizeof(TdqCtrl)];
     constexpr int kWords = (int)(sizeof(TdqCtrl) / 8);
     unsigned long long *sw = reinterpret_cast<unsigned long long *>(raw);
@@ -311,7 +313,7 @@
     __syncthreads();
     unsigned long long *go = reinterpret_cast<unsigned long long *>(c);
     for (int i = threadIdx.x; i < kWords; i += THREADS) go[i] = sw[i];
-    if (threadIdx.x == 0 && sc.loop_handle != 0ull)
+    if (set_cond && threadIdx.x == 0 && sc.loop_handle != 0ull)
         cudaGraphSetConditional((cudaGraphConditionalHandle)sc.loop_handle, sc.halt ? 0u : 1u);
 }
 
diff --git a/torchdiffeq_b200/odeint.py b/torchdiffeq_b200/odeint.py
--- a/torchdiffeq_b200/odeint.py
+++ b/torchdiffeq_b200/odeint.py
@@ -21,7 +21,8 @@
                      "max_num_steps", "dtype", "norm"}
 _FIXED_OPTIONS = {"step_size", "grid_constructor", "interp", "perturb", "norm"}
 _ADAMS_OPTIONS = _FIXED_OPTIONS | {"max_iters", "max_order"}
-_OUR_OPTIONS = {"graph", "run_ahead", "process_group", "cache", "exchange", "device_loop", "fused_linear", "fused_attempt", "fused_controller"}
+_OUR_OPTIONS = {"graph", "run_ahead", "process_group", "cache", "exchange", "device_loop", "fused_linear", "fused_attempt", "fused_controller",
+                "fused_loop"}
 
 
 def _rms_norm(tensor):
@@ -268,7 +269,8 @@
         from .fields import fusable
         w = fusable(getattr(p, "original_func", None), tuple(p.shape), p.dtype, p.device, eng.lib)
         if w is not None:
-            eng.set_linear(w, whole_attempt=o.get("fused_attempt", True), fused_controller=o.get("fused_controller", True))
+            eng.set_linear(w, whole_attempt=o.get("fused_attempt", True), fused_controller=o.get("fused_controller", True),
+                           fused_loop=o.get("fused_loop", True))
     return eng
 
 
@@ -667,4 +669,5 @@
         _stats["attempts"] = getattr(eng, "n_attempts", None)
         _stats["n_accept"], _stats["n_reject"] = getattr(eng, "n_accept", None), getattr(eng, "n_reject", None)
         _stats["fused_linear"], _stats["fused_attempt"] = _LAST_STATS["fused_linear"], _LAST_STATS["fused_attempt"]
+        _stats["fused_loop"] = bool(getattr(eng, "ran_fused_loop", False))
     return _unflatten(p, sol)
```

Result: faster. 8.920 million (median of 6 runs) (+11.0%).
